# hi-paris/Prosody-Control-French-TTS

Measured on AMD Instinct MI355X. Metric: audio-seconds/sec prosody+align throughput, 16 kHz French, higher is better.
Workload: dtype fp16-resid16 (MFMA legs) + f64 (F0 / LUFS)

## Files before the change

include/pce.h:

```cpp
#ifndef PCE_H
#define PCE_H

#include <stddef.h>
#include <stdint.h>

#ifdef __cplusplus
extern "C" {
#endif

#pragma GCC visibility push(default)

#define PCE_API_VERSION 1
#define PCE_API_MINOR 6

typedef struct pce_ctx pce_ctx;

enum pce_status {
    PCE_OK = 0,
    PCE_E_INVALID = -1,
    PCE_E_DEVICE = -2,
    PCE_E_NOMEM = -3,
    PCE_E_STATE = -4,
    PCE_E_LIMIT = -5
};

enum pce_slice_status {
    PCE_SLICE_OK = 0,
    PCE_SLICE_TOO_SHORT = 1,
    PCE_SLICE_EMPTY = 2
};

typedef struct pce_slice {
    int32_t clip;
    int32_t flags;
    int64_t begin;
    int64_t end;
    double  x1;
} pce_slice;


pce_ctx *pce_create(int device, void *stream, char *err, size_t errlen);
void pce_destroy(pce_ctx *ctx);
const char *pce_last_error(const pce_ctx *ctx);
int pce_sync(pce_ctx *ctx);
int pce_api_version(void);
int pce_api_minor(void);
int pce_device_info(pce_ctx *ctx, char *name, size_t namelen, int32_t *compute_units, int64_t *hbm_bytes);

int pce_upload_pcm_s16(pce_ctx *ctx, const int16_t *pcm, const int64_t *offsets, int32_t n_clips, int32_t sample_rate);
int pce_bind_pcm_s16_device(pce_ctx *ctx, const void *d_pcm, const int64_t *offsets, int32_t n_clips, int32_t sample_rate);
int pce_num_clips(const pce_ctx *ctx);

int pce_resample_run(pce_ctx *ctx, int32_t up, int32_t down, const double *taps, int32_t n_taps, int64_t n_pre_remove);
int pce_download_pcm_s16(pce_ctx *ctx, int16_t *pcm, int64_t *offsets, int32_t *sample_rate);

int pce_frame_energy_run(pce_ctx *ctx, int32_t window, int32_t hop, int32_t requantize);
int pce_frame_energy_shape(pce_ctx *ctx, int32_t clip, int64_t *n_frames);
int pce_frame_energy_fetch(pce_ctx *ctx, int32_t clip, int64_t *sum_sq , int32_t *count );

typedef struct pce_energy {
    int64_t n;
    int64_t sum_sq;
    int64_t sum_sq_wrap16;
    int64_t n_loud;
    int32_t peak_abs;
    int32_t reserved;
} pce_energy;
int pce_energy_run(pce_ctx *ctx, const pce_slice *slices, int32_t n_slices, int32_t loud_threshold);
int pce_energy_fetch(pce_ctx *ctx, pce_energy *out );

int pce_lufs_set_meter_rate(pce_ctx *ctx, int32_t rate);
int pce_lufs_run(pce_ctx *ctx, const pce_slice *slices, int32_t n_slices);
int pce_lufs_fetch(pce_ctx *ctx, double *lufs , int32_t *status );

typedef struct pce_pitch_params {
    double  time_step;
    double  pitch_floor;
    double  periods_per_window;
    int32_t max_candidates;
    int32_t reserved;
    double  silence_threshold;
    double  voicing_threshold;
    double  octave_cost;
    double  octave_jump_cost;
    double  voiced_unvoiced_cost;
    double  pitch_ceiling;
} pce_pitch_params;

typedef struct pce_pitch_summary {
    int64_t n_frames;
    int64_t n_voiced;
    double  median_f0;
    double  mean_log_f0;
    double  t1;
    int32_t status;
    int32_t reserved;
} pce_pitch_summary;

int pce_pitch_plan(pce_ctx *ctx, const pce_pitch_params *p, const pce_slice *slices, int32_t n_slices,
                   int64_t *frame_offsets, int32_t *status);
int pce_pitch_run(pce_ctx *ctx, const pce_pitch_params *p, const pce_slice *slices, int32_t n_slices);
enum { PCE_REFINE_SEEDED = 0, PCE_REFINE_PRAAT = 1 };
int pce_pitch_set_refine(pce_ctx *ctx, int32_t mode);
int pce_pitch_fetch(pce_ctx *ctx, double *f0, double *strength, pce_pitch_summary *summary );

int pce_stft_db_run(pce_ctx *ctx, int32_t n_fft, int32_t hop);
int pce_stft_db_shape(pce_ctx *ctx, int32_t clip, int32_t *n_bins, int32_t *n_frames);
int pce_stft_db_fetch(pce_ctx *ctx, int32_t clip, float *out);
int pce_stft_db_device(pce_ctx *ctx, const void **d_ptr, int64_t *bytes);

typedef struct pce_pyin_plan {
    int32_t frame_length, hop_length, min_period, max_period, n_pitch_bins, trans_width, n_thresholds, reserved;
    double sr, fmin, bins_per_octave, no_trough_prob, log_tiny, log_p_init, tiny;
} pce_pyin_plan;
int pce_pyin_run(pce_ctx *ctx, const pce_pyin_plan *plan, const double *tables, int64_t n_tables);
int pce_pyin_shape(pce_ctx *ctx, int32_t clip, int64_t *n_frames);
int pce_pyin_fetch(pce_ctx *ctx, int32_t clip, int32_t *states, double *voiced_prob, int32_t *status);

typedef struct pce_whisper_dims {
    int32_t n_mels;
    int32_t n_ctx;
    int32_t n_state;
    int32_t n_head;
    int32_t n_layer;
} pce_whisper_dims;
int pce_logmel_run(pce_ctx *ctx, int32_t n_mels);
int pce_logmel_run_at(pce_ctx *ctx, int32_t n_mels, const int64_t *start_frames );
int pce_logmel_fetch(pce_ctx *ctx, int32_t clip, float *out );
int pce_whisper_load(pce_ctx *ctx, const pce_whisper_dims *dims, const float *weights, int64_t n_floats);
int pce_whisper_encode_run(pce_ctx *ctx);
int pce_selftest_gemm(pce_ctx *ctx, const uint16_t *A, const uint16_t *B, const float *bias, int32_t M, int32_t N, int32_t K, int32_t epilogue,
                      int32_t rows_per_clip, int32_t vt_sp, uint16_t *out);
int pce_selftest_attention(pce_ctx *ctx, const uint16_t *q, const uint16_t *k, const uint16_t *v, int32_t clips, int32_t heads, int32_t q_len,
                           int32_t k_len, int32_t causal, int32_t mode, uint16_t *out, int32_t *fell_back);
int pce_selftest_xattn(pce_ctx *ctx, const float *resid, const float *ln_w, const float *ln_b, const uint16_t *wq, const float *bq, const uint16_t *wk,
                       const uint16_t *wv, const float *bv, const uint16_t *E, const int32_t *k_len, int32_t n, int32_t k_cap, int32_t d, int32_t heads,
                       int32_t workgroups_per_clip, uint16_t *out);
int pce_selftest_gemm_tiled(pce_ctx *ctx, int32_t kernel, int32_t epilogue, const uint16_t *A, int64_t a_len, int64_t lda, int64_t a_batch, int32_t batch,
                            const uint16_t *B, const float *bias, int32_t M, int32_t N, int32_t K, void *C, int64_t c_len, int64_t ldc, int64_t c_batch,
                            const float *pos, int32_t pos_T, int32_t v_col0, int32_t rows_per_clip, int32_t vt_sp, uint16_t *vt, int64_t vt_len,
                            int32_t *kernel_used);
int pce_selftest_layernorm(pce_ctx *ctx, int32_t form, int32_t rows, int32_t d, const void *x, const uint16_t *delta, const uint16_t *delta2, const float *w,
                           const float *b, float eps, int32_t flags, void *out, void *resid_out, uint16_t *out_copy);
int pce_whisper_encode_fetch(pce_ctx *ctx, int32_t clip, float *out );

typedef struct pce_whisper_text_dims {
    int32_t n_vocab , n_text_ctx , n_state, n_head , n_layer;
} pce_whisper_text_dims;
int pce_whisper_decoder_load(pce_ctx *ctx, const pce_whisper_text_dims *dims, const float *weights, int64_t n_floats);
int pce_whisper_align_run(pce_ctx *ctx, const int32_t *tokens, const int32_t *token_offsets, const int32_t *num_frames,
                          int32_t sot_len, const uint8_t *head_mask, int32_t medfilt_width, float qk_scale);
int pce_whisper_align_shape(pce_ctx *ctx, int32_t clip, int32_t *n_rows, int32_t *n_cols);
int pce_whisper_align_fetch(pce_ctx *ctx, int32_t clip, int32_t *text_idx, int32_t *time_idx, int32_t *path_len, double *cost);
int pce_whisper_align_paths_enqueue(pce_ctx *ctx, int32_t slot, int32_t *n_clips, int32_t *path_stride);
int pce_whisper_align_paths_wait(pce_ctx *ctx, int32_t slot, int32_t *path_len, int32_t *text_idx, int32_t *time_idx);

typedef struct pce_whisper_decode_rules { int32_t eot, timestamp_begin, max_initial_timestamp_index , reserved; } pce_whisper_decode_rules;
int pce_whisper_decode_step(pce_ctx *ctx, const int32_t *tokens, const int32_t *token_offsets , int32_t sample_begin,
                            const pce_whisper_decode_rules *rules, const uint8_t *vocab_mask, int32_t *next_tokens ,
                            float *next_logprobs );
typedef struct pce_whisper_decode_opts {
    const int32_t *sample_begin;
    int32_t sample_begin_all;
    float temperature;
    uint32_t seed_lo, seed_hi;
    int32_t probe_token;
    int32_t flags;
} pce_whisper_decode_opts;
int pce_whisper_decode_step_ex(pce_ctx *ctx, const int32_t *tokens, const int32_t *token_offsets ,
                               const pce_whisper_decode_rules *rules, const uint8_t *vocab_mask, const pce_whisper_decode_opts *opts,
                               int32_t *next_tokens , float *next_logprobs ,
                               float *probe_prob );

int pce_whisper_sample_keys(pce_ctx *ctx, const int32_t *keys , int32_t n);

enum { PCE_OPERANDS_BF16 = 0, PCE_OPERANDS_FP16 = 1, PCE_OPERANDS_F16_RESID16 = 2 };
int pce_whisper_set_operands(pce_ctx *ctx, int32_t operand_type);
int pce_whisper_get_operands(pce_ctx *ctx);

int pce_whisper_decode_loop(pce_ctx *ctx, const int32_t *tokens, const int32_t *token_offsets ,
                            const pce_whisper_decode_rules *rules, const uint8_t *vocab_mask, const pce_whisper_decode_opts *opts,
                            int32_t max_new, int32_t check_every, int32_t *out_tokens, float *out_logprobs ,
                            int32_t *out_steps, float *probe_prob );

int pce_dtw(pce_ctx *ctx, const double *x, int32_t n_rows, int32_t n_cols, int32_t batch, int32_t *path_i, int32_t *path_j,
            int32_t *path_len);

#define PCE_DTW_SERIES_ROWS 1024
#define PCE_DTW_SERIES_COLS 2048
enum pce_dtw_status { PCE_DTW_OK = 0, PCE_DTW_EMPTY = 1, PCE_DTW_NO_PATH = 2 };
int pce_dtw_series(pce_ctx *ctx, const double *a, const int64_t *a_off, const double *b, const int64_t *b_off, const int32_t *win_lo,
                   const int32_t *win_hi, int32_t batch, int32_t *path_i, int32_t *path_j, int32_t *path_len, double *dist, int32_t *status);

int pce_nw_align(pce_ctx *ctx, const int32_t *a_ids, const int64_t *a_off, const int32_t *b_ids, const int64_t *b_off, int32_t batch,
                 int32_t match, int32_t mismatch, int32_t gap, int32_t *out_i, int32_t *out_j, int32_t *out_len);

int pce_levenshtein(pce_ctx *ctx, const uint32_t *a_chars, const int64_t *a_off, const uint32_t *b_chars, const int64_t *b_off,
                    int32_t batch, int32_t *out_dist);

typedef struct pce_bert_dims { int32_t n_vocab, n_pos, n_type, n_state, n_head, n_layer, n_labels; } pce_bert_dims;
int pce_bert_load(pce_ctx *ctx, const pce_bert_dims *dims, const float *weights, int64_t n_floats);
int pce_bert_run(pce_ctx *ctx, const int32_t *input_ids, const int32_t *offsets , int32_t n_seq);
int pce_bert_fetch(pce_ctx *ctx, int32_t seq, float *logits, int32_t *labels);

int pce_stats_enqueue(pce_ctx *ctx, int32_t slot);
int pce_stats_wait(pce_ctx *ctx, int32_t slot, pce_energy *energy, double *lufs, int32_t *lufs_status, pce_pitch_summary *pitch);

enum pce_kernel_id {
    PCE_K_ENERGY = 0,
    PCE_K_LUFS_PASS1, PCE_K_LUFS_SCAN, PCE_K_LUFS_PASS2, PCE_K_LUFS_GATE,
    PCE_K_PITCH_REFINE, PCE_K_PITCH_FRAMES, PCE_K_PITCH_PATH, PCE_K_PITCH_MEDIAN, PCE_K_PITCH_DELTA,
    PCE_K_STFT_MAX, PCE_K_STFT_DB, PCE_K_LOGMEL, PCE_K_WHISPER_ENC, PCE_K_RESAMPLE, PCE_K_DTW, PCE_K_WHISPER_ALIGN, PCE_K_NW, PCE_K_STFT_NORM,
    PCE_K_FRAME_ENERGY, PCE_K_BERT, PCE_K_PYIN_FRAMES, PCE_K_PYIN_VITERBI, PCE_K_WHISPER_DECODE,
    PCE_K_GEMM128, PCE_K_GEMM_WIDE, PCE_K_ATTENTION, PCE_K_LAYERNORM, PCE_K_GEMM_FLAT,
    PCE_K_ADD_LAYERNORM, PCE_K_STFT_RAW, PCE_K_LOGMEL_NORM, PCE_K_ATTENTION_LEAN,
// ... 17 lines not shown
```

prosody-control-french-tts_amd/csrc/pce_gemm256.inc:

```

constexpr int F_T = 256, F_K = 64, F_THREADS = 512;
constexpr int F_N_MAX = 6144;
constexpr bool F_PINGPONG = true;
constexpr int F_HALF = 128 * F_K;
constexpr int F_RING_BYTES = 8 * F_HALF * 2;
enum { FEPI_BF16 = 0, FEPI_GELU = 1, FEPI_VT = 2, FEPI_SPLIT = 3 };

__device__ __forceinline__ int f_swz(int row, int chunk) { return chunk ^ ((row >> 1) & 7); }
__device__ __forceinline__ int f_perm32(int p) { return ((p >> 2) & 3) * 8 + (p >> 4) * 4 + (p & 3); }

struct FCursor { int kofs, m0, n0, vt; };
struct FSched {
    int tiles_n, sm, sn, per_xcd, xcd, slot, wper, my_tiles;
    __device__ void init(int M, int N, int sm_, int sn_)
    {
        tiles_n = N / F_T; sm = sm_; sn = sn_;
        const int tiles_m = (M + F_T - 1) / F_T, tiles_m_pad = ((tiles_m + sm - 1) / sm) * sm;
        const int total = tiles_m_pad * tiles_n;
        per_xcd = (total + 7) >> 3; xcd = blockIdx.x & 7; slot = blockIdx.x >> 3; wper = gridDim.x >> 3;
        my_tiles = per_xcd > slot ? (per_xcd - slot + wper - 1) / wper : 0;
    }
    __device__ void tile(int it, int &m0, int &n0) const
    {
        const int lin = xcd * per_xcd + slot + it * wper;
        const int per = sm * sn, sup = lin / per, r = lin - sup * per;
        const int n_sn = tiles_n / sn;
        m0 = ((sup / n_sn) * sm + r / sn) * F_T; n0 = ((sup % n_sn) * sn + r % sn) * F_T;
    }
};

struct FFrags { opx8 RA[2][4], RB0[2][2], RB1[2][2]; };
struct FArgs {
    const op_t *A, *B; const float *bias; op_t *C;
    int M, N, K, ldc;
    int S, vt_sp;
    int sm, sn, stagger;
    op_t *C2; int vt_n0;
};

template <int N> __device__ __forceinline__ void f_wait_vm() { __builtin_amdgcn_s_waitcnt(((N >> 4) << 14) | 0x0F70 | (N & 15)); }
template <int N> __device__ __forceinline__ void f_wait_lgkm() { __builtin_amdgcn_s_waitcnt(0xC07F | (N << 8)); }

template <int KK, int HALF>
__device__ __forceinline__ void f_read_A(FFrags &F, const op_t *dsm, const int (&ra)[2], int par)
{
    const op_t *s = dsm + ((HALF ? 1 : 0) * 2 + par) * F_HALF;
#pragma unroll
    for (int i = 0; i < 4; i++) F.RA[KK][i] = *reinterpret_cast<const opx8 *>(s + ra[KK] + i * 16 * F_K);
}
template <int KK, int HALF>
__device__ __forceinline__ void f_read_B(FFrags &F, const op_t *dsm, const int (&rb)[2], int par)
{
    const op_t *s = dsm + ((HALF ? 1 : 0) * 2 + par) * F_HALF;
#pragma unroll
    for (int j = 0; j < 2; j++) {
        const opx8 v = *reinterpret_cast<const opx8 *>(s + rb[KK] + j * 16 * F_K);
        if (HALF) F.RB1[KK][j] = v; else F.RB0[KK][j] = v;
    }
}
template <bool VT, int HA, int HB, int KK, bool ZERO>
__device__ __forceinline__ void f_mma8(f32x4 (&acc)[2][2][4][2], const FFrags &F)
{
#pragma unroll
    for (int i = 0; i < 4; i++)
#pragma unroll
        for (int j = 0; j < 2; j++) {
            const opx8 b = HB ? F.RB1[KK][j] : F.RB0[KK][j];
            const f32x4 c = ZERO ? f32x4{0.f, 0.f, 0.f, 0.f} : acc[HA][HB][i][j];
            acc[HA][HB][i][j] = VT ? mfma16(F.RA[KK][i], b, c)
                                   : mfma16(b, F.RA[KK][i], c);
        }
}

template <int EPI>
__global__ __launch_bounds__(F_THREADS) __attribute__((amdgpu_waves_per_eu(2, 2))) void k_gemm_flat(FArgs P)
{
    constexpr bool SPLIT = EPI == FEPI_SPLIT;
    extern __shared__ __attribute__((aligned(1024))) op_t dsm[];
    float *sbias = reinterpret_cast<float *>(dsm + 8 * F_HALF);
    const int tid = threadIdx.x, lane = tid & 63, wv = __builtin_amdgcn_readfirstlane(tid >> 6);
    const int wr = wv >> 2, wc = wv & 3;
    const int fr = lane & 15, fq = lane >> 4;
    const int M = P.M, N = P.N, K = P.K;
    FSched S; S.init(M, N, P.sm, P.sn);
    const int nk = K / F_K;
    if (S.my_tiles == 0) return;
    for (int i = tid; i < N; i += F_THREADS) sbias[i] = P.bias ? P.bias[i] : 0.f;
    if (P.stagger > 0) {
        const unsigned long long t0 = __builtin_amdgcn_s_memtime(), d = (unsigned long long)P.stagger * (unsigned)(S.slot * 8 + S.xcd) / 256u;
        while (__builtin_amdgcn_s_memtime() - t0 < d) __builtin_amdgcn_s_sleep(8);
    }
    int voff_plain, voff_perm;
    {
        const int row = wv * 8 + (lane >> 3), c8 = f_swz(row, lane & 7) * 8;
        const int prow = (row & ~31) + f_perm32(row & 31);
        voff_plain = (row * K + c8) * 2; voff_perm = (prow * K + c8) * 2;
    }
    int ra[2], rb[2];
    {
        const int r_a = wr * 64 + fr, r_b = wc * 32 + fr;
        ra[0] = r_a * F_K + f_swz(r_a, fq) * 8; ra[1] = r_a * F_K + f_swz(r_a, 4 + fq) * 8;
        rb[0] = r_b * F_K + f_swz(r_b, fq) * 8 + 4 * F_HALF; rb[1] = r_b * F_K + f_swz(r_b, 4 + fq) * 8 + 4 * F_HALF;
    }
    const __amdgpu_buffer_rsrc_t rsA = __builtin_amdgcn_make_buffer_rsrc(const_cast<op_t *>(P.A), 0, (int)((unsigned)M * (unsigned)K * 2u), 0x00020000);
    const __amdgpu_buffer_rsrc_t rsB = __builtin_amdgcn_make_buffer_rsrc(const_cast<op_t *>(P.B), 0, (int)((unsigned)N * (unsigned)K * 2u), 0x00020000);
    const int ld2_64 = 64 * K * 2;
    FCursor pc1, pc2;
    int it1, kt1, it2, kt2;
    const int last_tile = S.my_tiles - 1;
    auto set_tile = [&](FCursor &c, int it) {
        S.tile(it < last_tile ? it : last_tile, c.m0, c.n0);
        c.vt = SPLIT ? (c.n0 >= P.vt_n0) : (EPI == FEPI_VT);
    };
    auto advance = [&](FCursor &c, int &it, int &kt) {
        if (++kt == nk) { kt = 0; ++it; set_tile(c, it); }
        c.kofs = kt * F_K;
    };
    auto issue = [&](const FCursor &c, int kind, int par) {
        op_t *slot = dsm + ((kind == 0 ? 0 : kind == 3 ? 1 : kind == 1 ? 2 : 3) * 2 + par) * F_HALF;
        const bool is_a = kind == 0 || kind == 3;
        const bool act = SPLIT ? (is_a != (c.vt != 0)) : is_a;
        const unsigned soff = (unsigned)((act ? c.m0 : c.n0) + ((kind == 3 || kind == 2) ? 128 : 0)) * (unsigned)K * 2u + (unsigned)c.kofs * 2u;
        const int voff = ((EPI == FEPI_VT) == is_a) ? voff_perm : voff_plain;
#pragma unroll
        for (int i = 0; i < 2; i++)
            __builtin_amdgcn_raw_ptr_buffer_load_lds(act ? rsA : rsB, (__attribute__((address_space(3))) void *)(slot + (wv + 8 * i) * 8 * F_K), 16,
                                                     voff, (int)(soff + (unsigned)(i * ld2_64)), 0, 0);
    };
    f32x4 acc[2][2][4][2];
#pragma unroll
    for (int a = 0; a < 2; a++)
#pragma unroll
        for (int b = 0; b < 2; b++)
#pragma unroll
            for (int i = 0; i < 4; i++)
#pragma unroll
                for (int j = 0; j < 2; j++) acc[a][b][i][j] = f32x4{0.f, 0.f, 0.f, 0.f};
    FFrags F;

#ifndef F_STORE_AUX
#define F_STORE_AUX 0
#endif
#define F_STORE_GUARD { asm volatile("s_nop 7\n\ts_nop 7" ::: "memory"); __builtin_amdgcn_sched_barrier(0); }
    typedef unsigned int u32x4 __attribute__((ext_vector_type(4)));
    constexpr bool HAS_RM = EPI != FEPI_VT, HAS_VT = EPI == FEPI_VT || SPLIT;
    const int Nv = SPLIT ? N - P.vt_n0 : N;
    op_t *const vt_ptr = SPLIT ? P.C2 : P.C;
    const __amdgpu_buffer_rsrc_t rsC = __builtin_amdgcn_make_buffer_rsrc(P.C, 0, HAS_RM ? (int)((unsigned)M * (unsigned)P.ldc * 2u) : 0, 0x00020000);
    const __amdgpu_buffer_rsrc_t rsV = __builtin_amdgcn_make_buffer_rsrc(vt_ptr, 0, HAS_VT ? (int)((unsigned)(M / P.S) * (unsigned)Nv * (unsigned)P.vt_sp * 2u) : 0, 0x00020000);
    const int voffC = (fr * P.ldc + fq * 8) * 2, voffV = (fr * P.vt_sp + fq * 8) * 2;
    auto store_rm = [&](int m0, int n0) {
#pragma unroll
        for (int hB = 0; hB < 2; hB++) {
            const float *bp = sbias + n0 + hB * 128 + wc * 32 + fq * 8;
            const float4 b0 = *reinterpret_cast<const float4 *>(bp), b1 = *reinterpret_cast<const float4 *>(bp + 4);
            const float bv[8] = {b0.x, b0.y, b0.z, b0.w, b1.x, b1.y, b1.z, b1.w};
#pragma unroll
            for (int hA = 0; hA < 2; hA++)
#pragma unroll
                for (int i = 0; i < 4; i++) {
                    opx8 o;
                    float t[8];
#pragma unroll
                    for (int e = 0; e < 8; e++) t[e] = acc[hA][hB][i][e >> 2][e & 3] + bv[e];
                    if (EPI == FEPI_GELU) gelu_exact8(t);
#pragma unroll
                    for (int e = 0; e < 8; e++) o[e] = (op_t)t[e];
                    const unsigned soff = ((unsigned)(m0 + hA * 128 + wr * 64 + i * 16) * (unsigned)P.ldc + (unsigned)(n0 + hB * 128 + wc * 32)) * 2u;
                    __builtin_amdgcn_raw_buffer_store_b128(__builtin_bit_cast(u32x4, o), rsC, voffC, (int)soff, F_STORE_AUX);
                    __builtin_amdgcn_sched_barrier(0);
                    F_STORE_GUARD
                }
        }
    };
    auto store_vt = [&](int m0, int n0, int nb0) {
        typedef __attribute__((ext_vector_type(4))) op_t opx4;
        typedef unsigned int u32x2 __attribute__((ext_vector_type(2)));
        const int clip0 = m0 / P.S, t_tile = m0 - clip0 * P.S;
        const int wrap = (Nv * P.vt_sp - P.S) * 2;
#pragma unroll
        for (int hB = 0; hB < 2; hB++)
#pragma unroll
            for (int j = 0; j < 2; j++) {
                const int n_s = n0 + hB * 128 + wc * 32 + j * 16;
                const float bv = sbias[nb0 + hB * 128 + wc * 32 + j * 16 + fr];
                const unsigned col = ((unsigned)clip0 * (unsigned)Nv + (unsigned)n_s) * (unsigned)P.vt_sp;
#pragma unroll
                for (int hA = 0; hA < 2; hA++)
#pragma unroll
                    for (int g = 0; g < 2; g++) {
                        const int t_g = t_tile + hA * 128 + wr * 64 + g * 32, rel = P.S - t_g;
                        if (!(rel > 0 && rel < 32 && (rel & 7) == 4)) {
                            opx8 o;
#pragma unroll
                            for (int r = 0; r < 8; r++) o[r] = (op_t)(acc[hA][hB][2 * g + (r >> 2)][j][r & 3] + bv);
                            const int voff = voffV + ((t_g + fq * 8 >= P.S) ? wrap : 0);
                            __builtin_amdgcn_raw_buffer_store_b128(__builtin_bit_cast(u32x4, o), rsV, voff, (int)((col + (unsigned)t_g) * 2u), F_STORE_AUX);
                            F_STORE_GUARD
                        } else {
#pragma unroll
                            for (int h = 0; h < 2; h++) {
                                const int t_s = t_g + h * 4;
                                opx4 o;
#pragma unroll
                                for (int r = 0; r < 4; r++) o[r] = (op_t)(acc[hA][hB][2 * g + h][j][r] + bv);
                                const int voff = voffV + ((t_s + fq * 8 >= P.S) ? wrap : 0);
                                __builtin_amdgcn_raw_buffer_store_b64(__builtin_bit_cast(u32x2, o), rsV, voff, (int)((col + (unsigned)t_s) * 2u), F_STORE_AUX);
                                F_STORE_GUARD
                            }
                        }
                    }
                __builtin_amdgcn_sched_barrier(0);
            }
    };
    auto store_vtT = [&](int m0, int n0) {
        typedef __attribute__((ext_vector_type(4))) op_t opx4;
        typedef unsigned int u32x2 __attribute__((ext_vector_type(2)));
        const int clip0 = m0 / P.S, t_tile = m0 - clip0 * P.S;
        const int wrap = (Nv * P.vt_sp - P.S) * 2;
#pragma unroll
        for (int hB = 0; hB < 2; hB++) {
            const int t_g = t_tile + hB * 128 + wc * 32, rel = P.S - t_g;
            const bool cut = rel > 0 && rel < 32 && (rel & 7) == 4;
#pragma unroll
            for (int hA = 0; hA < 2; hA++)
#pragma unroll
                for (int i = 0; i < 4; i++) {
                    const int n_r = hA * 128 + wr * 64 + i * 16;
                    const float bv = sbias[n0 + n_r + fr];
                    const unsigned base = (((unsigned)clip0 * (unsigned)Nv + (unsigned)(n0 - P.vt_n0 + n_r)) * (unsigned)P.vt_sp + (unsigned)t_g) * 2u;
                    if (!cut) {
                        opx8 o;
#pragma unroll
                        for (int e = 0; e < 8; e++) o[e] = (op_t)(acc[hA][hB][i][e >> 2][e & 3] + bv);
                        const int voff = voffV + ((t_g + fq * 8 >= P.S) ? wrap : 0);
                        __builtin_amdgcn_raw_buffer_store_b128(__builtin_bit_cast(u32x4, o), rsV, voff, (int)base, F_STORE_AUX);
                        F_STORE_GUARD
                    } else {
#pragma unroll
                        for (int h = 0; h < 2; h++) {
                            opx4 o;
#pragma unroll
                            for (int r = 0; r < 4; r++) o[r] = (op_t)(acc[hA][hB][i][h][r] + bv);
                            const int voff = voffV + h * 8 + ((t_g + fq * 8 + h * 4 >= P.S) ? wrap : 0);
                            __builtin_amdgcn_raw_buffer_store_b64(__builtin_bit_cast(u32x2, o), rsV, voff, (int)base, F_STORE_AUX);
                            F_STORE_GUARD
                        }
                    }
                    __builtin_amdgcn_sched_barrier(0);
                }
// ... 1 lines not shown
    };
    constexpr int EPI_OPS = 16;

    {
        FCursor c0; c0.kofs = 0; set_tile(c0, 0);
        it1 = 0; kt1 = 0; pc1 = c0; advance(pc1, it1, kt1);
        it2 = it1; kt2 = kt1; pc2 = pc1; advance(pc2, it2, kt2);
        __syncthreads();
        issue(c0, 0, 0); issue(c0, 1, 0); issue(c0, 2, 0); issue(c0, 3, 0);
        issue(pc1, 0, 1); issue(pc1, 1, 1); issue(pc1, 2, 1);
        f_wait_vm<6>();
        __builtin_amdgcn_s_barrier();
        if constexpr (!F_PINGPONG) {
            f_read_A<0, 0>(F, dsm, ra, 0); f_read_B<0, 0>(F, dsm, rb, 0); f_read_B<0, 1>(F, dsm, rb, 0); f_read_B<1, 1>(F, dsm, rb, 0);
            f_wait_lgkm<0>();
        }
    }
    int c_m0, c_n0;
    S.tile(0, c_m0, c_n0);
    int par = 0;
#define F_GROUP(HA, HB, KK) __builtin_amdgcn_s_setprio(1); f_mma8<VT, HA, HB, KK, false>(acc, F); \
                             __builtin_amdgcn_s_setprio(0); __builtin_amdgcn_sched_barrier(0);
#define F_ISSUE(C, KIND, PAR) __builtin_amdgcn_sched_barrier(0); issue(C, KIND, PAR); __builtin_amdgcn_sched_barrier(0);
    constexpr bool VT = EPI == FEPI_VT;
    auto kstep = [&](bool first_stores) {
        __builtin_amdgcn_s_barrier();
        F_ISSUE(pc1, 3, par ^ 1)
        f_read_A<1, 0>(F, dsm, ra, par); f_read_B<1, 0>(F, dsm, rb, par);
        f_wait_lgkm<6>(); F_GROUP(0, 0, 0)
        F_GROUP(0, 1, 0)
        f_read_A<0, 1>(F, dsm, ra, par);
        f_wait_lgkm<4>(); F_GROUP(0, 0, 1)
        F_GROUP(0, 1, 1)
        if (first_stores) f_wait_vm<2 + EPI_OPS>(); else f_wait_vm<2>();
        f_wait_lgkm<0>();
        __builtin_amdgcn_s_barrier();
        F_ISSUE(pc2, 0, par)
        f_read_A<1, 1>(F, dsm, ra, par);
        f_wait_lgkm<4>(); F_GROUP(1, 1, 0)
        F_ISSUE(pc2, 1, par)
        f_read_B<0, 1>(F, dsm, rb, par ^ 1);
        f_wait_lgkm<2>(); F_GROUP(1, 0, 0)
        F_ISSUE(pc2, 2, par)
        f_read_A<0, 0>(F, dsm, ra, par ^ 1); f_read_B<0, 0>(F, dsm, rb, par ^ 1);
        f_wait_lgkm<6>(); F_GROUP(1, 1, 1)
        f_read_B<1, 1>(F, dsm, rb, par ^ 1);
        f_wait_lgkm<2>(); F_GROUP(1, 0, 1)
    };
    auto kstep_pp = [&](int after_stores) {
        f_read_A<0, 0>(F, dsm, ra, par); f_read_A<1, 0>(F, dsm, ra, par); f_read_B<0, 0>(F, dsm, rb, par); f_read_B<1, 0>(F, dsm, rb, par);
        F_ISSUE(pc1, 3, par ^ 1)
        f_wait_lgkm<0>();
        __builtin_amdgcn_s_barrier();
        F_GROUP(0, 0, 0) F_GROUP(0, 0, 1)
        __builtin_amdgcn_s_barrier();
        f_read_B<0, 1>(F, dsm, rb, par); f_read_B<1, 1>(F, dsm, rb, par);
        F_ISSUE(pc2, 0, par)
        if (after_stores == 2) f_wait_vm<10>();
        f_wait_lgkm<0>();
        __builtin_amdgcn_s_barrier();
        F_GROUP(0, 1, 0) F_GROUP(0, 1, 1)
        __builtin_amdgcn_s_barrier();
        f_read_A<0, 1>(F, dsm, ra, par); f_read_A<1, 1>(F, dsm, ra, par);
        F_ISSUE(pc2, 1, par)
        f_wait_lgkm<0>();
        __builtin_amdgcn_s_barrier();
        F_GROUP(1, 1, 0) F_GROUP(1, 1, 1)
        __builtin_amdgcn_s_barrier();
        F_ISSUE(pc2, 2, par)
        if (after_stores == 1) f_wait_vm<8 + EPI_OPS>(); else f_wait_vm<6>();
        __builtin_amdgcn_s_barrier();
        F_GROUP(1, 0, 0) F_GROUP(1, 0, 1)
        __builtin_amdgcn_s_barrier();
    };
    if (F_PINGPONG && wr == 1) __builtin_amdgcn_s_barrier();
    for (int it = 0; it < S.my_tiles; it++) {
        const bool cur_vt = SPLIT ? (c_n0 >= P.vt_n0) : (EPI == FEPI_VT);
        for (int kt = 0; kt < nk; kt++) {
            const bool first = kt == 0, last = kt == nk - 1;
            if constexpr (F_PINGPONG) kstep_pp(it > 0 && nk >= 2 ? (kt == 0 ? 1 : kt == 1 ? 2 : 0) : 0);
            else kstep(first && it > 0);
            pc1 = pc2; it1 = it2; kt1 = kt2; advance(pc2, it2, kt2);
            if (last) {
                if (F_PINGPONG && wr == 0) __builtin_amdgcn_s_barrier();
                if constexpr (SPLIT) { if (cur_vt) store_vtT(c_m0, c_n0); else store_rm(c_m0, c_n0); }
                else if constexpr (EPI == FEPI_VT) store_vt(c_m0, c_n0, c_n0);
                else store_rm(c_m0, c_n0);
                if constexpr (!F_PINGPONG) f_wait_vm<6 + EPI_OPS>();
#pragma unroll
                for (int a = 0; a < 2; a++)
#pragma unroll
                    for (int b = 0; b < 2; b++)
#pragma unroll
                        for (int i = 0; i < 4; i++)
#pragma unroll
                            for (int j = 0; j < 2; j++) acc[a][b][i][j] = f32x4{0.f, 0.f, 0.f, 0.f};
                if (F_PINGPONG && wr == 1) __builtin_amdgcn_s_barrier();
            } else if constexpr (!F_PINGPONG) f_wait_vm<6>();
            f_wait_lgkm<0>();
            par ^= 1;
        }
        if (it + 1 < S.my_tiles) S.tile(it + 1, c_m0, c_n0);
    }
    if (F_PINGPONG && wr == 0) __builtin_amdgcn_s_barrier();
    f_wait_vm<0>();
#undef F_GROUP
#undef F_ISSUE
#undef F_STORE_GUARD
}

template <class OUT, class RIN, class ROUT, int NV = 5>
__global__ __launch_bounds__(256) void k_add_layernorm(const RIN *resid_in, ROUT *resid_out, const op_t *__restrict__ delta, const op_t *__restrict__ delta2,
                                                      int write_resid, const float *__restrict__ w,
                                                      const float *__restrict__ b, int64_t rows, int d, OUT *__restrict__ out, float eps,
                                                      op_t *__restrict__ out_bf16 = nullptr )
{
    constexpr bool IN16 = !std::is_same<RIN, float>::value, OUT16 = !std::is_same<ROUT, float>::value;
    const int64_t row = (int64_t)blockIdx.x * 4 + (threadIdx.x >> 6);
    const int lane = threadIdx.x & 63;
    if (row >= rows) return;
    typedef __attribute__((ext_vector_type(4))) op_t opx4;
    const opx4 *dr = reinterpret_cast<const opx4 *>(delta + row * d);
    const opx4 *dr2 = reinterpret_cast<const opx4 *>(delta2 ? delta2 + row * d : nullptr);
    auto r16 = [](float x) -> float { return OUT16 ? (float)(op_t)x : x; };
    const int nv = d >> 2;
    float4 v[NV];
    float s = 0.f;
#pragma unroll
    for (int i = 0; i < NV; i++) {
        const int idx = lane + 64 * i;
        if (idx < nv) {
            f32x4 x;
            if constexpr (IN16) {
                const opx4 xh = __builtin_nontemporal_load(reinterpret_cast<const opx4 *>(resid_in + row * d) + idx);
                x = f32x4{(float)xh[0], (float)xh[1], (float)xh[2], (float)xh[3]};
            } else {
                x = __builtin_nontemporal_load(reinterpret_cast<const f32x4 *>(resid_in + row * d) + idx);
                if constexpr (OUT16) x = f32x4{r16(x[0]), r16(x[1]), r16(x[2]), r16(x[3])};
            }
            const opx4 dl = __builtin_nontemporal_load(dr + idx);
            v[i] = make_float4(r16(x[0] + (float)dl[0]), r16(x[1] + (float)dl[1]), r16(x[2] + (float)dl[2]), r16(x[3] + (float)dl[3]));
            if (dr2) {
                const opx4 d2 = __builtin_nontemporal_load(dr2 + idx);
                v[i] = make_float4(r16(v[i].x + (float)d2[0]), r16(v[i].y + (float)d2[1]), r16(v[i].z + (float)d2[2]), r16(v[i].w + (float)d2[3]));
            }
            if (write_resid) {
                if constexpr (OUT16) {
                    opx4 o; o[0] = (op_t)v[i].x; o[1] = (op_t)v[i].y; o[2] = (op_t)v[i].z; o[3] = (op_t)v[i].w;
                    __builtin_nontemporal_store(o, reinterpret_cast<opx4 *>(resid_out + row * d) + idx);
                } else __builtin_nontemporal_store(f32x4{v[i].x, v[i].y, v[i].z, v[i].w}, reinterpret_cast<f32x4 *>(resid_out + row * d) + idx);
            }
        } else v[i] = make_float4(0.f, 0.f, 0.f, 0.f);
        s += (v[i].x + v[i].y) + (v[i].z + v[i].w);
    }
    s = wave_allsum_f32(s);
    const float mean = s / (float)d;
    float q = 0.f;
#pragma unroll
    for (int i = 0; i < NV; i++) {
        if (lane + 64 * i < nv) {
            const float a0 = v[i].x - mean, a1 = v[i].y - mean, a2 = v[i].z - mean, a3 = v[i].w - mean;
            q += (a0 * a0 + a1 * a1) + (a2 * a2 + a3 * a3);
        }
    }
    q = wave_allsum_f32(q);
    const float inv = rsqrtf(q / (float)d + eps);
// ... 13 lines not shown
```

prosody-control-french-tts_amd/csrc/pce_whisper_dispatch.hip:

```cpp
#include "pce_internal.h"

#define PCE_BOTH(ret, name, params)  extern "C" { ret name##_bf16 params; ret name##_f16 params; }
#define PCE_FWD(name, ...) ((c && c->whisper_ops >= 1) ? name##_f16(__VA_ARGS__) : name##_bf16(__VA_ARGS__))

PCE_BOTH(int, pce_logmel_run, (pce_ctx *, int32_t))
PCE_BOTH(int, pce_logmel_run_at, (pce_ctx *, int32_t, const int64_t *))
PCE_BOTH(int, pce_logmel_fetch, (pce_ctx *, int32_t, float *))
PCE_BOTH(int, pce_whisper_load, (pce_ctx *, const pce_whisper_dims *, const float *, int64_t))
PCE_BOTH(int, pce_whisper_encode_run, (pce_ctx *))
PCE_BOTH(int, pce_whisper_encode_fetch, (pce_ctx *, int32_t, float *))
PCE_BOTH(int, pce_selftest_attention, (pce_ctx *, const uint16_t *, const uint16_t *, const uint16_t *, int32_t, int32_t, int32_t, int32_t, int32_t, int32_t, uint16_t *, int32_t *))
PCE_BOTH(int, pce_selftest_gemm, (pce_ctx *, const uint16_t *, const uint16_t *, const float *, int32_t, int32_t, int32_t, int32_t, int32_t, int32_t, uint16_t *))
PCE_BOTH(int, pce_selftest_xattn, (pce_ctx *, const float *, const float *, const float *, const uint16_t *, const float *, const uint16_t *, const uint16_t *, const float *, const uint16_t *, const int32_t *, int32_t, int32_t, int32_t, int32_t, int32_t, uint16_t *))
PCE_BOTH(int, pce_selftest_gemm_tiled, (pce_ctx *, int32_t, int32_t, const uint16_t *, int64_t, int64_t, int64_t, int32_t, const uint16_t *, const float *, int32_t, int32_t,
                                         int32_t, void *, int64_t, int64_t, int64_t, const float *, int32_t, int32_t, int32_t, int32_t, uint16_t *, int64_t, int32_t *))
PCE_BOTH(int, pce_selftest_layernorm, (pce_ctx *, int32_t, int32_t, int32_t, const void *, const uint16_t *, const uint16_t *, const float *, const float *, float, int32_t,
                                        void *, void *, uint16_t *))
PCE_BOTH(int, pce_whisper_decoder_load, (pce_ctx *, const pce_whisper_text_dims *, const float *, int64_t))
PCE_BOTH(int, pce_whisper_align_run, (pce_ctx *, const int32_t *, const int32_t *, const int32_t *, int32_t, const uint8_t *, int32_t, float))
PCE_BOTH(int, pce_whisper_align_fetch, (pce_ctx *, int32_t, int32_t *, int32_t *, int32_t *, double *))
PCE_BOTH(int, pce_whisper_align_shape, (pce_ctx *, int32_t, int32_t *, int32_t *))
PCE_BOTH(int, pce_whisper_align_paths_enqueue, (pce_ctx *, int32_t, int32_t *, int32_t *))
PCE_BOTH(int, pce_whisper_align_paths_wait, (pce_ctx *, int32_t, int32_t *, int32_t *, int32_t *))
PCE_BOTH(int, pce_whisper_sample_keys, (pce_ctx *, const int32_t *, int32_t))
PCE_BOTH(int, pce_whisper_decode_step, (pce_ctx *, const int32_t *, const int32_t *, int32_t, const pce_whisper_decode_rules *, const uint8_t *, int32_t *, float *))
PCE_BOTH(int, pce_whisper_decode_step_ex, (pce_ctx *, const int32_t *, const int32_t *, const pce_whisper_decode_rules *, const uint8_t *, const pce_whisper_decode_opts *, int32_t *, float *, float *))
PCE_BOTH(int, pce_whisper_decode_loop, (pce_ctx *, const int32_t *, const int32_t *, const pce_whisper_decode_rules *, const uint8_t *, const pce_whisper_decode_opts *, int32_t, int32_t, int32_t *, float *, int32_t *, float *))
PCE_BOTH(int, pce_bert_load, (pce_ctx *, const pce_bert_dims *, const float *, int64_t))
PCE_BOTH(int, pce_bert_run, (pce_ctx *, const int32_t *, const int32_t *, int32_t))
PCE_BOTH(int, pce_bert_fetch, (pce_ctx *, int32_t, float *, int32_t *))
void pce_whisper_free_bf16(pce_ctx *c);
void pce_whisper_free_f16(pce_ctx *c);

void pce_whisper_free(pce_ctx *c) { pce_whisper_free_bf16(c); pce_whisper_free_f16(c); }

extern "C" {

int pce_whisper_set_operands(pce_ctx *c, int32_t operand_type)
{
    if (!c) return PCE_E_INVALID;
    if (operand_type != PCE_OPERANDS_BF16 && operand_type != PCE_OPERANDS_FP16 && operand_type != PCE_OPERANDS_F16_RESID16)
        return pce_fail(c, PCE_E_INVALID, "operand type %d (0 = bf16, 1 = fp16, 2 = fp16 with the fp16 residual stream)", operand_type);
    c->whisper_ops = operand_type;
    c->resid16 = operand_type == PCE_OPERANDS_F16_RESID16;
    return PCE_OK;
}
int pce_whisper_get_operands(pce_ctx *c) { return c ? c->whisper_ops : PCE_E_INVALID; }

int pce_logmel_run(pce_ctx *c, int32_t n_mels) { return PCE_FWD(pce_logmel_run, c, n_mels); }
int pce_logmel_run_at(pce_ctx *c, int32_t n_mels, const int64_t *start_frames) { return PCE_FWD(pce_logmel_run_at, c, n_mels, start_frames); }
int pce_logmel_fetch(pce_ctx *c, int32_t clip, float *out) { return PCE_FWD(pce_logmel_fetch, c, clip, out); }
int pce_whisper_load(pce_ctx *c, const pce_whisper_dims *dims, const float *weights, int64_t n_floats) { return PCE_FWD(pce_whisper_load, c, dims, weights, n_floats); }
int pce_whisper_encode_run(pce_ctx *c) { return PCE_FWD(pce_whisper_encode_run, c); }
int pce_whisper_encode_fetch(pce_ctx *c, int32_t clip, float *out) { return PCE_FWD(pce_whisper_encode_fetch, c, clip, out); }
int pce_selftest_attention(pce_ctx *c, const uint16_t *q, const uint16_t *k, const uint16_t *v, int32_t clips, int32_t heads, int32_t q_len, int32_t k_len,
                           int32_t causal, int32_t mode, uint16_t *out, int32_t *fell_back)
{
    return PCE_FWD(pce_selftest_attention, c, q, k, v, clips, heads, q_len, k_len, causal, mode, out, fell_back);
}
int pce_selftest_gemm(pce_ctx *c, const uint16_t *A, const uint16_t *B, const float *bias, int32_t M, int32_t N, int32_t K, int32_t epilogue, int32_t rows_per_clip,
                      int32_t vt_sp, uint16_t *out)
{
    return PCE_FWD(pce_selftest_gemm, c, A, B, bias, M, N, K, epilogue, rows_per_clip, vt_sp, out);
}
int pce_selftest_xattn(pce_ctx *c, const float *resid, const float *ln_w, const float *ln_b, const uint16_t *wq, const float *bq, const uint16_t *wk, const uint16_t *wv,
                       const float *bv, const uint16_t *E, const int32_t *k_len, int32_t n, int32_t k_cap, int32_t d, int32_t heads, int32_t workgroups_per_clip, uint16_t *out)
{
    return PCE_FWD(pce_selftest_xattn, c, resid, ln_w, ln_b, wq, bq, wk, wv, bv, E, k_len, n, k_cap, d, heads, workgroups_per_clip, out);
}
int pce_selftest_gemm_tiled(pce_ctx *c, int32_t kernel, int32_t epilogue, const uint16_t *A, int64_t a_len, int64_t lda, int64_t a_batch, int32_t batch,
                            const uint16_t *B, const float *bias, int32_t M, int32_t N, int32_t K, void *C, int64_t c_len, int64_t ldc, int64_t c_batch,
                            const float *pos, int32_t pos_T, int32_t v_col0, int32_t rows_per_clip, int32_t vt_sp, uint16_t *vt, int64_t vt_len, int32_t *kernel_used)
{
    return PCE_FWD(pce_selftest_gemm_tiled, c, kernel, epilogue, A, a_len, lda, a_batch, batch, B, bias, M, N, K, C, c_len, ldc, c_batch, pos, pos_T, v_col0,
                   rows_per_clip, vt_sp, vt, vt_len, kernel_used);
}
int pce_selftest_layernorm(pce_ctx *c, int32_t form, int32_t rows, int32_t d, const void *x, const uint16_t *delta, const uint16_t *delta2, const float *w,
                           const float *b, float eps, int32_t flags, void *out, void *resid_out, uint16_t *out_copy)
{
    return PCE_FWD(pce_selftest_layernorm, c, form, rows, d, x, delta, delta2, w, b, eps, flags, out, resid_out, out_copy);
}
int pce_whisper_decoder_load(pce_ctx *c, const pce_whisper_text_dims *dims, const float *weights, int64_t n_floats)
{
    return PCE_FWD(pce_whisper_decoder_load, c, dims, weights, n_floats);
}
int pce_whisper_align_run(pce_ctx *c, const int32_t *tokens, const int32_t *token_offsets, const int32_t *num_frames, int32_t sot_len, const uint8_t *head_mask,
                          int32_t medfilt_width, float qk_scale)
{
    return PCE_FWD(pce_whisper_align_run, c, tokens, token_offsets, num_frames, sot_len, head_mask, medfilt_width, qk_scale);
}
int pce_whisper_align_fetch(pce_ctx *c, int32_t clip, int32_t *text_idx, int32_t *time_idx, int32_t *path_len, double *cost)
{
    return PCE_FWD(pce_whisper_align_fetch, c, clip, text_idx, time_idx, path_len, cost);
}
int pce_whisper_align_shape(pce_ctx *c, int32_t clip, int32_t *n_rows, int32_t *n_cols) { return PCE_FWD(pce_whisper_align_shape, c, clip, n_rows, n_cols); }
int pce_whisper_align_paths_enqueue(pce_ctx *c, int32_t slot, int32_t *n_clips, int32_t *path_stride) { return PCE_FWD(pce_whisper_align_paths_enqueue, c, slot, n_clips, path_stride); }
int pce_whisper_align_paths_wait(pce_ctx *c, int32_t slot, int32_t *path_len, int32_t *text_idx, int32_t *time_idx)
{
    return PCE_FWD(pce_whisper_align_paths_wait, c, slot, path_len, text_idx, time_idx);
}
int pce_whisper_sample_keys(pce_ctx *c, const int32_t *keys, int32_t n) { return PCE_FWD(pce_whisper_sample_keys, c, keys, n); }
int pce_whisper_decode_step(pce_ctx *c, const int32_t *tokens, const int32_t *token_offsets, int32_t sample_begin, const pce_whisper_decode_rules *rules,
                            const uint8_t *vocab_mask, int32_t *next_tokens, float *next_logprobs)
{
    return PCE_FWD(pce_whisper_decode_step, c, tokens, token_offsets, sample_begin, rules, vocab_mask, next_tokens, next_logprobs);
}
int pce_whisper_decode_step_ex(pce_ctx *c, const int32_t *tokens, const int32_t *token_offsets, const pce_whisper_decode_rules *rules, const uint8_t *vocab_mask,
                               const pce_whisper_decode_opts *opts, int32_t *next_tokens, float *next_logprobs, float *probe_prob)
{
    return PCE_FWD(pce_whisper_decode_step_ex, c, tokens, token_offsets, rules, vocab_mask, opts, next_tokens, next_logprobs, probe_prob);
}
int pce_whisper_decode_loop(pce_ctx *c, const int32_t *tokens, const int32_t *token_offsets, const pce_whisper_decode_rules *rules, const uint8_t *vocab_mask,
                            const pce_whisper_decode_opts *opts, int32_t max_new, int32_t check_every, int32_t *out_tokens, float *out_logprobs, int32_t *out_steps,
                            float *probe_prob)
{
    return PCE_FWD(pce_whisper_decode_loop, c, tokens, token_offsets, rules, vocab_mask, opts, max_new, check_every, out_tokens, out_logprobs, out_steps, probe_prob);
}
int pce_bert_load(pce_ctx *c, const pce_bert_dims *dims, const float *weights, int64_t n_floats) { return PCE_FWD(pce_bert_load, c, dims, weights, n_floats); }
int pce_bert_run(pce_ctx *c, const int32_t *input_ids, const int32_t *offsets, int32_t n_seq) { return PCE_FWD(pce_bert_run, c, input_ids, offsets, n_seq); }
int pce_bert_fetch(pce_ctx *c, int32_t seq, float *logits, int32_t *labels) { return PCE_FWD(pce_bert_fetch, c, seq, logits, labels); }

}
```

prosody-control-french-tts_amd/csrc/pce_whisper_impl.inc:

```
#include "pce_internal.h"
#include <cmath>
#include <cstdlib>
#include <type_traits>

#define pce_logmel_run PCE_WFN(pce_logmel_run)
#define pce_logmel_run_at PCE_WFN(pce_logmel_run_at)
#define pce_logmel_fetch PCE_WFN(pce_logmel_fetch)
#define pce_whisper_load PCE_WFN(pce_whisper_load)
#define pce_whisper_encode_run PCE_WFN(pce_whisper_encode_run)
#define pce_whisper_encode_fetch PCE_WFN(pce_whisper_encode_fetch)
#define pce_selftest_attention PCE_WFN(pce_selftest_attention)
#define pce_selftest_gemm PCE_WFN(pce_selftest_gemm)
#define pce_whisper_decoder_load PCE_WFN(pce_whisper_decoder_load)
#define pce_whisper_align_run PCE_WFN(pce_whisper_align_run)
#define pce_whisper_align_fetch PCE_WFN(pce_whisper_align_fetch)
#define pce_whisper_align_shape PCE_WFN(pce_whisper_align_shape)
#define pce_whisper_align_paths_enqueue PCE_WFN(pce_whisper_align_paths_enqueue)
#define pce_whisper_align_paths_wait PCE_WFN(pce_whisper_align_paths_wait)
#define pce_whisper_sample_keys PCE_WFN(pce_whisper_sample_keys)
#define pce_whisper_decode_step PCE_WFN(pce_whisper_decode_step)
#define pce_whisper_decode_step_ex PCE_WFN(pce_whisper_decode_step_ex)
#define pce_whisper_decode_loop PCE_WFN(pce_whisper_decode_loop)
#define pce_bert_load PCE_WFN(pce_bert_load)
#define pce_bert_run PCE_WFN(pce_bert_run)
#define pce_bert_fetch PCE_WFN(pce_bert_fetch)
#define pce_selftest_xattn PCE_WFN(pce_selftest_xattn)
#define pce_selftest_gemm_tiled PCE_WFN(pce_selftest_gemm_tiled)
#define pce_selftest_layernorm PCE_WFN(pce_selftest_layernorm)
#define pce_whisper_free PCE_WFN(pce_whisper_free)
extern "C" int pce_whisper_decode_step_ex(pce_ctx *c, const int32_t *tokens, const int32_t *token_offsets, const pce_whisper_decode_rules *rules,
                                          const uint8_t *vocab_mask, const pce_whisper_decode_opts *opts, int32_t *next_tokens,
                                          float *next_logprobs, float *probe_prob);
void pce_whisper_free(pce_ctx *c);

namespace {

typedef PCE_OP_T op_t;
typedef __attribute__((ext_vector_type(8))) op_t opx8;
typedef __attribute__((ext_vector_type(4))) float f32x4;

template <class T> struct MfmaOf;
template <> struct MfmaOf<__bf16> {
    typedef __attribute__((ext_vector_type(8))) __bf16 v8;
    static __device__ __forceinline__ f32x4 m16(v8 a, v8 b, f32x4 c) { return __builtin_amdgcn_mfma_f32_16x16x32_bf16(a, b, c, 0, 0, 0); }
};
template <> struct MfmaOf<_Float16> {
    typedef __attribute__((ext_vector_type(8))) _Float16 v8;
    static __device__ __forceinline__ f32x4 m16(v8 a, v8 b, f32x4 c) { return __builtin_amdgcn_mfma_f32_16x16x32_f16(a, b, c, 0, 0, 0); }
};
__device__ __forceinline__ f32x4 mfma16(opx8 a, opx8 b, f32x4 c) { return MfmaOf<op_t>::m16(a, b, c); }

constexpr int W_NFFT = 400, W_HOP = 160, W_BINS = 201, W_FRAMES = 3000, W_SAMPLES = 480000;
constexpr int W_CTX = 1500;
constexpr double W_PI = 3.14159265358979323846;

struct MelTables {
    const float2 *w16;
    const float2 *w400;
    const float2 *w25;
    const float *window;
    const int *mel_lo;
    const int *mel_n;
    const int *mel_off;
    const float *mel_w;
    int mel_total;
};

__device__ __forceinline__ unsigned int f32_order_key(float f)
{
    const unsigned int b = __float_as_uint(f);
    return (b & 0x80000000u) ? ~b : (b | 0x80000000u);
}
__device__ __forceinline__ float f32_from_key(unsigned int k)
{
    return __uint_as_float((k & 0x80000000u) ? (k & 0x7FFFFFFFu) : ~k);
}

constexpr int LM_MELW = 1024;
template <int LM_G>
__global__ __launch_bounds__(256) PCE_NO_PK_F32 void k_logmel_frames(const int16_t *__restrict__ pcm, const int64_t *__restrict__ clip_off, int n_mels,
                                                      MelTables T, float *__restrict__ logspec ,
                                                      unsigned int *__restrict__ clip_max, const int64_t *__restrict__ frame0, int scan)
{
    __shared__ float xs[4][W_NFFT];
    __shared__ float2 ys[4][25 * 16];
    __shared__ float pw[4][W_BINS + 3];
    __shared__ float2 s_w16[16], s_w25[25], s_w400[25 * 16];
    __shared__ float s_melw[LM_MELW];
    const int tid = threadIdx.x, lane = tid & 63, wv = tid >> 6;
    for (int i = tid; i < T.mel_total; i += 256) s_melw[i] = T.mel_w[i];
    for (int i = tid; i < 16; i += 256) s_w16[i] = T.w16[i];
    for (int i = tid; i < 25; i += 256) s_w25[i] = T.w25[i];
    for (int i = tid; i < 400; i += 256) s_w400[i] = T.w400[i];
    __syncthreads();
    const int clip = blockIdx.y;
// ... 502 lines not shown
#pragma unroll
    for (int s = 0; s < W_STAGES - 1; s++)
        if (s < nk) {
            stage_rows32<G_BM>(A, lda, m0, M - 1, s * W_BK, smem + s * W_STAGE, wv, lane);
            stage_rows32<W_BN>(B, K, n0, N - 1, s * W_BK, smem + s * W_STAGE + G_BM * W_BK, wv, lane);
        }
    int cur = 0;
    for (int kt = 0; kt < nk; kt++) {
        const op_t *sA = smem + cur * W_STAGE, *sB = sA + G_BM * W_BK;
        if (W_STAGES > 2 && kt + 1 < nk) asm volatile("s_waitcnt vmcnt(3)" ::: "memory");
        else asm volatile("s_waitcnt vmcnt(0)" ::: "memory");
        __builtin_amdgcn_s_barrier();
        if (kt + W_STAGES - 1 < nk) {
            int nx = cur + W_STAGES - 1; if (nx >= W_STAGES) nx -= W_STAGES;
            op_t *nA = smem + nx * W_STAGE;
            stage_rows32<G_BM>(A, lda, m0, M - 1, (kt + W_STAGES - 1) * W_BK, nA, wv, lane);
            stage_rows32<W_BN>(B, K, n0, N - 1, (kt + W_STAGES - 1) * W_BK, nA + G_BM * W_BK, wv, lane);
        }
        opx8 a[4], b[4];
#pragma unroll
        for (int i = 0; i < 4; i++) {
            const int row = wr * 64 + i * 16 + fr;
            a[i] = *reinterpret_cast<const opx8 *>(&sA[row * W_BK + swz32(row, fq) * 8]);
        }
#pragma unroll
        for (int j = 0; j < 4; j++) {
            const int row = wc * 64 + j * 16 + fr;
            b[j] = *reinterpret_cast<const opx8 *>(&sB[row * W_BK + swz32(row, fq) * 8]);
        }
#pragma unroll
        for (int i = 0; i < 4; i++)
#pragma unroll
            for (int j = 0; j < 4; j++) acc[i][j] = mfma16(a[i], b[j], acc[i][j]);
        cur = cur + 1 == W_STAGES ? 0 : cur + 1;
    }
    float *tile = reinterpret_cast<float *>(smem);
#pragma unroll
    for (int p = 0; p < 2; p++) {
        __syncthreads();
        if ((wc >> 1) == p) {
#pragma unroll
            for (int i = 0; i < 4; i++)
#pragma unroll
                for (int j = 0; j < 4; j++)
#pragma unroll
                    for (int r = 0; r < 4; r++)
                        tile[(wr * 64 + i * 16 + fq * 4 + r) * G_TLD + (wc & 1) * 64 + j * 16 + fr] = acc[i][j][r];
        }
        __syncthreads();
        if (p == 0) gemm_store_tile<EPI>(tile, tid, m0, n0, M, N, bv0, bc0, Cv, ldc, (int64_t)blockIdx.z * c_batch, pos, pos_T, v_col0, vt_sp);
        else gemm_store_tile<EPI>(tile, tid, m0, n0 + 128, M, N, bv1, bc1, Cv, ldc, (int64_t)blockIdx.z * c_batch, pos, pos_T, v_col0, vt_sp);
    }
}

template <class OUT> __device__ __forceinline__ void ln_store4(OUT *p, float a, float b, float c, float d);
template <> __device__ __forceinline__ void ln_store4<float>(float *p, float a, float b, float c, float d)
{
    *reinterpret_cast<float4 *>(p) = make_float4(a, b, c, d);
}
template <> __device__ __forceinline__ void ln_store4<op_t>(op_t *p, float a, float b, float c, float d)
{
    typedef __attribute__((ext_vector_type(4))) op_t opx4;
    opx4 v; v[0] = (op_t)a; v[1] = (op_t)b; v[2] = (op_t)c; v[3] = (op_t)d;
    *reinterpret_cast<opx4 *>(p) = v;
}

template <int CTRL> __device__ __forceinline__ float dpp_f32(float v)
{
    return __builtin_bit_cast(float, __builtin_amdgcn_update_dpp(0, __builtin_bit_cast(int, v), CTRL, 0xF, 0xF, true));
}
__device__ __forceinline__ float wave_allsum_f32(float v)
{
    v += dpp_f32<0xB1>(v);
    v += dpp_f32<0x4E>(v);
    v += dpp_f32<0x141>(v);
    v += dpp_f32<0x140>(v);
    const int b = __builtin_bit_cast(int, v);
    const float r0 = __builtin_bit_cast(float, __builtin_amdgcn_readlane(b, 0)), r1 = __builtin_bit_cast(float, __builtin_amdgcn_readlane(b, 16));
    const float r2 = __builtin_bit_cast(float, __builtin_amdgcn_readlane(b, 32)), r3 = __builtin_bit_cast(float, __builtin_amdgcn_readlane(b, 48));
    return (r0 + r1) + (r2 + r3);
}

constexpr int LN_D_MAX = 2048;
template <class OUT, int NV = 5>
__global__ __launch_bounds__(256) void k_layernorm(const float *x, const float *__restrict__ w, const float *__restrict__ b,
                                                  int64_t rows, int d, OUT *__restrict__ out, float eps = 1e-5f, float *out2 = nullptr, int round_in16 = 0)
{
    const int64_t row = (int64_t)blockIdx.x * 4 + (threadIdx.x >> 6);
    const int lane = threadIdx.x & 63;
    if (row >= rows) return;
    const float4 *xr = reinterpret_cast<const float4 *>(x + row * d);
    const int nv = d >> 2;
    float4 v[NV];
    float s = 0.f;
#pragma unroll
    for (int i = 0; i < NV; i++) {
        const int idx = lane + 64 * i;
        v[i] = idx < nv ? xr[idx] : make_float4(0.f, 0.f, 0.f, 0.f);
        if (round_in16) v[i] = make_float4((float)(op_t)v[i].x, (float)(op_t)v[i].y, (float)(op_t)v[i].z, (float)(op_t)v[i].w);
        s += (v[i].x + v[i].y) + (v[i].z + v[i].w);
    }
    s = wave_allsum_f32(s);
    const float mean = s / (float)d;
    float q = 0.f;
#pragma unroll
    for (int i = 0; i < NV; i++) {
        if (lane + 64 * i < nv) {
            const float a0 = v[i].x - mean, a1 = v[i].y - mean, a2 = v[i].z - mean, a3 = v[i].w - mean;
            q += (a0 * a0 + a1 * a1) + (a2 * a2 + a3 * a3);
        }
    }
    q = wave_allsum_f32(q);
    const float inv = rsqrtf(q / (float)d + eps);
#pragma unroll
    for (int i = 0; i < NV; i++) {
        const int idx = lane + 64 * i;
        if (idx < nv) {
            const float4 ww = reinterpret_cast<const float4 *>(w)[idx], bb = reinterpret_cast<const float4 *>(b)[idx];
            const float y0 = (v[i].x - mean) * inv * ww.x + bb.x, y1 = (v[i].y - mean) * inv * ww.y + bb.y,
                        y2 = (v[i].z - mean) * inv * ww.z + bb.z, y3 = (v[i].w - mean) * inv * ww.w + bb.w;
            ln_store4<OUT>(out + row * d + 4 * idx, y0, y1, y2, y3);
            if (out2) ln_store4<float>(out2 + row * d + 4 * idx, y0, y1, y2, y3);
        }
    }
}

#include "pce_gemm256.inc"

constexpr int AT_QB = 128;

struct AttnArgs {
    const op_t *q; int64_t q_ld;
    const op_t *k; int64_t k_ld;
    const op_t *vt; int64_t vt_clip; int vt_sp;
    const int *q_row0, *q_len, *k_row0, *k_len;
    op_t *out; int64_t out_ld;
    int causal;
    int *fell_back;
};

template <bool EXACT, bool NT>
__device__ __forceinline__ bool attn_block16(const AttnArgs &A, op_t *smem, int bx, int head, int clip)
{
    constexpr int NS = 3, DPW = 4;
    const int tid = threadIdx.x, lane = tid & 63, wv = __builtin_amdgcn_readfirstlane(tid >> 6);
    const int n16 = lane & 15, g = lane >> 4;
    const int Sq = A.q_len[clip], Sk = A.k_len[clip];
    const int q0 = bx * AT_QB + wv * 32;
    const op_t *qbase = A.q + (int64_t)A.q_row0[clip] * A.q_ld + head * 64;
    const op_t *kbase = A.k + (int64_t)A.k_row0[clip] * A.k_ld + head * 64;
    const op_t *vtbase = A.vt + (int64_t)clip * A.vt_clip + (int64_t)head * 64 * A.vt_sp;
    const int kld = (int)A.k_ld, vsp = A.vt_sp;
    const __amdgpu_buffer_rsrc_t rsK = __builtin_amdgcn_make_buffer_rsrc(const_cast<op_t *>(kbase), 0, ((Sk - 1) * kld + 64) * 2, 0x00020000);
    const __amdgpu_buffer_rsrc_t rsV = __builtin_amdgcn_make_buffer_rsrc(const_cast<op_t *>(vtbase), 0, 64 * vsp * 2, 0x00020000);
    int voffK[2], voffV[2];
#pragma unroll
    for (int i = 0; i < 2; i++) {
        const int row = (wv + 4 * i) * 8 + (lane >> 3), c8 = swz_chunk(row, lane & 7) * 8;
        const int kb = row >> 4, rho = row & 15;
        const int key = 32 * (kb >> 1) + 8 * (rho >> 2) + 4 * (kb & 1) + (rho & 3);
        voffK[i] = (key * kld + c8) * 2; voffV[i] = (row * vsp + c8) * 2;
    }
    auto stage = [&](int t) {
        op_t *sK = smem + (t % NS) * (2 * 64 * 64), *sV = sK + 64 * 64;
        const int key0 = t * 64;
#pragma unroll
        for (int i = 0; i < 2; i++) {
            __builtin_amdgcn_raw_ptr_buffer_load_lds(rsK, (__attribute__((address_space(3))) void *)(sK + (wv + 4 * i) * 8 * 64), 16, voffK[i], key0 * kld * 2, 0, NT ? 3 : 0);
            __builtin_amdgcn_raw_ptr_buffer_load_lds(rsV, (__attribute__((address_space(3))) void *)(sV + (wv + 4 * i) * 8 * 64), 16, voffV[i], key0 * 2, 0, NT ? 3 : 0);
        }
    };
    const f32x4 z4 = {0.f, 0.f, 0.f, 0.f};
    opx8 qf[2][2];
    int my_q[2];
#pragma unroll
    for (int qb = 0; qb < 2; qb++) {
        my_q[qb] = q0 + 16 * qb + n16;
        int qr = my_q[qb]; if (qr >= Sq) qr = Sq - 1;
        const op_t *qp = qbase + (int64_t)qr * A.q_ld;
#pragma unroll
        for (int ks = 0; ks < 2; ks++) qf[qb][ks] = *reinterpret_cast<const opx8 *>(qp + 32 * ks + 8 * g);
    }
    opx8 ones;
#pragma unroll
    for (int j = 0; j < 8; j++) ones[j] = (op_t)(n16 == 0 ? 1.0f : 0.0f);
    f32x4 o[4][2], osum[2];
#pragma unroll
    for (int db = 0; db < 4; db++) { o[db][0] = z4; o[db][1] = z4; }
    osum[0] = z4; osum[1] = z4;
    float m_run[2] = {-1e30f, -1e30f}, l_run[2] = {0.f, 0.f};
    const float sl2 = 0.125f * 1.4426950408889634f;
    int k_need = Sk;
    if (A.causal) k_need = min(Sk, bx * AT_QB + AT_QB);
    const int nt = (k_need + 63) / 64;
    int kaddr[4][2], vaddr[4][2];
#pragma unroll
    for (int b4 = 0; b4 < 4; b4++)
#pragma unroll
        for (int ks = 0; ks < 2; ks++) {
            const int row = 16 * b4 + n16;
            kaddr[b4][ks] = row * 64 + swz_chunk(row, 4 * ks + g) * 8;
            vaddr[b4][ks] = 64 * 64 + row * 64 + swz_chunk(row, 4 * ks + g) * 8;
        }
    stage(0);
    if (nt > 1) stage(1);
// ... 925 lines not shown
    P.sn = 1;
    for (int cand : {4, 3, 2}) if (tiles_n % cand == 0) { P.sn = cand; break; }
    const int tiles_m = (M + F_T - 1) / F_T;
    int sm_want = 16;
    P.stagger = 20000;
    if (tiles_n == 3 && K <= 1024) { P.sn = 1; sm_want = 8; }
    else if (tiles_n == 6) P.sn = tiles_n;
    P.sm = tiles_m < sm_want ? tiles_m : sm_want;
    const int lds = F_RING_BYTES + N * (int)sizeof(float);
    const int grid = ((c->cu_count > 0 ? c->cu_count : 256) / 8) * 8;
    KernelTimer kt(c, prof_id, nullptr, 2.0 * M * (double)N * K);
    hipLaunchKernelGGL((k_gemm_flat<EPI>), dim3((unsigned)grid), dim3(F_THREADS), lds, c->stream, P);
    return true;
}

enum GemmKernel { GK_AUTO = 0, GK_SKINNY = 1, GK_WIDE = 2, GK_128 = 3, GK_128_DEEP = 4 };
struct GemmShape { int M, N, K; int64_t lda; int batch; int v_col0; };
template <int EPI> static bool gemm_fits(int kind, const GemmShape &s)
{
    switch (kind) {
    case GK_SKINNY:
        return (EPI == EPI_BF16 || EPI == EPI_GELU_BF16 || EPI == EPI_RESID_F32) && s.batch == 1 && s.M <= 1024 && s.N <= 4096 && s.N % S_BN == 0 &&
               s.K % S_KC == 0 && s.lda % 8 == 0;
    case GK_WIDE: return s.N % W_BN == 0 && s.K % W_BK == 0 && (EPI != EPI_QKV || s.v_col0 % W_BN == 0);
    case GK_128: case GK_128_DEEP: return s.N % G_BN == 0 && s.K % G_BK == 0 && (EPI != EPI_QKV || s.v_col0 % G_BN == 0);
    default: return false;
    }
}
template <int EPI> static int gemm_choose(const pce_ctx *c, const GemmShape &s)
{
    if (c->gemm_skinny && c->gemm_few_rows && gemm_fits<EPI>(GK_SKINNY, s)) return GK_SKINNY;
    if (gemm_fits<EPI>(GK_WIDE, s) && s.N >= 1536 && !(EPI == EPI_F32 && (int64_t)s.M * s.batch <= 1024))
        return GK_WIDE;
    if ((int64_t)s.M * s.batch <= 1024 && s.K >= 4 * G_BK) return GK_128_DEEP;
    return GK_128;
}
template <int EPI>
static void launch_gemm_kernel(pce_ctx *c, int kind, const op_t *A, int64_t lda, int64_t a_batch, const op_t *B, int M, int N, int K, const float *bias,
                               void *C, int64_t ldc, int64_t c_batch, int batch, const float *pos, int pos_T, int v_col0, int vt_sp)
{
    if constexpr (EPI == EPI_BF16 || EPI == EPI_GELU_BF16 || EPI == EPI_RESID_F32) {
        if (kind == GK_SKINNY) {
            KernelTimer kt(c, PCE_K_GEMM_SKINNY, nullptr, 2.0 * M * (double)N * K);
            hipLaunchKernelGGL((k_gemm_skinny<EPI>), dim3((unsigned)(N / S_BN), (unsigned)div_up(M, S_BM)), dim3(S_THREADS), S_LDS, c->stream,
                               A, lda, B, M, N, K, bias, C, ldc);
            return;
        }
    }
    if (kind == GK_WIDE) {
        const int wt = N / W_BN;
        int wsn = 1;
        for (int cand : {4, 3, 2}) if (wt % cand == 0) { wsn = cand; break; }
        const int wsm = 16;
        dim3 wgrid((unsigned)wt, (unsigned)(div_up(M, G_BM * wsm) * wsm), (unsigned)batch);
        KernelTimer kt(c, PCE_K_GEMM_WIDE, nullptr, 2.0 * M * (double)N * K * batch);
        hipLaunchKernelGGL((k_gemm_wide<EPI>), wgrid, dim3(G_THREADS), 0, c->stream, A, lda, a_batch, B, M, N, K, bias, C, ldc, c_batch, pos, pos_T,
                           v_col0, vt_sp, wsn, wsm);
        return;
    }
    const int tiles_n = N / G_BN;
    int sn = 1;
    for (int cand : {8, 6, 4, 3, 2}) if (tiles_n % cand == 0) { sn = cand; break; }
    const int sm = 16;
    dim3 grid((unsigned)tiles_n, (unsigned)(div_up(M, G_BM * sm) * sm), (unsigned)batch);
    KernelTimer kt(c, PCE_K_GEMM128, nullptr, 2.0 * M * (double)N * K * batch);
    if (kind == GK_128_DEEP)
        hipLaunchKernelGGL((k_gemm_bf16<EPI, 4>), grid, dim3(G_THREADS), 0, c->stream, A, lda, a_batch, B, M, N, K, bias, C, ldc, c_batch, pos, pos_T,
                           v_col0, vt_sp, sn, sm);
    else
        hipLaunchKernelGGL((k_gemm_bf16<EPI>), grid, dim3(G_THREADS), 0, c->stream, A, lda, a_batch, B, M, N, K, bias, C, ldc, c_batch, pos, pos_T,
                           v_col0, vt_sp, sn, sm);
}
template <int EPI>
void launch_gemm(pce_ctx *c, const op_t *A, int64_t lda, int64_t a_batch, const op_t *B, int M, int N, int K, const float *bias,
                 void *C, int64_t ldc, int64_t c_batch, int batch, const float *pos = nullptr, int pos_T = 1, int v_col0 = 0,
                 int vt_sp = AT_SP)
{
    const int kind = gemm_choose<EPI>(c, GemmShape{M, N, K, lda, batch, v_col0});
    launch_gemm_kernel<EPI>(c, kind, A, lda, a_batch, B, M, N, K, bias, C, ldc, c_batch, batch, pos, pos_T, v_col0, vt_sp);
}

template <class OUT>
static void launch_layernorm(pce_ctx *c, const float *x, const float *w, const float *b, int64_t rows, int d, OUT *out, float eps = 1e-5f,
                             float *out2 = nullptr, int round_in16 = 0)
{
    const dim3 grid((unsigned)div_up(rows, 4)), block(256);
    if (d <= 1280) hipLaunchKernelGGL((k_layernorm<OUT, 5>), grid, block, 0, c->stream, x, w, b, rows, d, out, eps, out2, round_in16);
    else hipLaunchKernelGGL((k_layernorm<OUT, 8>), grid, block, 0, c->stream, x, w, b, rows, d, out, eps, out2, round_in16);
}
template <class OUT, class RIN, class ROUT>
static void launch_add_layernorm(pce_ctx *c, const RIN *resid_in, ROUT *resid_out, const op_t *delta, const op_t *delta2, int write_resid, const float *w,
                                 const float *b, int64_t rows, int d, OUT *out, float eps, op_t *out_bf16)
{
    const dim3 grid((unsigned)div_up(rows, 4)), block(256);
    if (d <= 1280)
        hipLaunchKernelGGL((k_add_layernorm<OUT, RIN, ROUT, 5>), grid, block, 0, c->stream, resid_in, resid_out, delta, delta2, write_resid, w, b, rows, d, out, eps, out_bf16);
    else
        hipLaunchKernelGGL((k_add_layernorm<OUT, RIN, ROUT, 8>), grid, block, 0, c->stream, resid_in, resid_out, delta, delta2, write_resid, w, b, rows, d, out, eps, out_bf16);
}

static bool xa_has_form(int d, int heads)
{
    return heads * 64 == d && (d == 128 || d == 256 || d == 384 || d == 512 || d == 768 || d == 1024 || d == 1280);
}
static int xa_split(int n, int wpc) { return (wpc == 1 || wpc == 2 || wpc == 4) ? wpc : n >= 512 ? 1 : n >= 256 ? 2 : 4; }
template <int D> struct XaWidth {
    static constexpr int NSLOT = (D == 512 || D == 768 || D == 1024) ? 2 : 3, WV = xa_waves(D), RT = D > 1024 ? 2 : 1;
    static constexpr bool PAIRS = D <= 768;
    static constexpr size_t LDS = xa_lds(D, NSLOT);
};
struct XaLayer {
    const float *resid, *ln_w, *ln_b, *bq, *bv;
    const op_t *wq, *wkT, *wv;
    op_t *qp_hi, *qp_lo, *out; int64_t out_ld;
};
template <int D>
static void xattn_launch_d(pce_ctx *c, int n, XaArgs a, const XaLayer &y)
{
    using W = XaWidth<D>;
    a.qp_hi = y.qp_hi; a.qp_lo = y.qp_lo;
    const dim3 hgrid((unsigned)a.heads, (unsigned)div_up(n, 16)), grid((unsigned)(n * a.nsplit)), block(64 * (unsigned)W::WV);
    hipLaunchKernelGGL(k_xq_fused<D>, hgrid, dim3(256), 0, c->stream, y.resid, y.ln_w, y.ln_b, y.wq, y.bq, y.wkT, n, 0.125f * 1.4426950408889634f, a.skip,
                       y.qp_hi, y.qp_lo, a.rows);
    auto uv = [&](auto kern) {
        hipLaunchKernelGGL(kern, hgrid, dim3(256), 0, c->stream, a.u_part, a.ml_part, y.wv, y.bv, n, a.skip, y.out, y.out_ld, a.rows);
    };
    if constexpr (W::PAIRS) {
        if (a.nsplit <= XA_LEAVES / 2) {
            hipLaunchKernelGGL((k_xattn_absorbed<D, W::NSLOT, true, W::WV, W::RT>), grid, block, W::LDS, c->stream, a);
            uv(k_uv_absorb<D, true>);
            return;
        }
    }
    hipLaunchKernelGGL((k_xattn_absorbed<D, W::NSLOT, false, W::WV, W::RT>), grid, block, W::LDS, c->stream, a);
    uv(k_uv_absorb<D, false>);
}
static void xattn_launch(pce_ctx *c, int d, int n, const XaArgs &a, const XaLayer &y)
{
    switch (d) {
    case 128: xattn_launch_d<128>(c, n, a, y); break;
    case 256: xattn_launch_d<256>(c, n, a, y); break;
    case 384: xattn_launch_d<384>(c, n, a, y); break;
    case 512: xattn_launch_d<512>(c, n, a, y); break;
    case 768: xattn_launch_d<768>(c, n, a, y); break;
    case 1024: xattn_launch_d<1024>(c, n, a, y); break;
    default: xattn_launch_d<1280>(c, n, a, y); break;
    }
}

template <int D> static hipError_t xattn_optin()
{
    using W = XaWidth<D>;
    if constexpr (W::PAIRS) {
        const hipError_t e = hipFuncSetAttribute((const void *)k_xattn_absorbed<D, W::NSLOT, true, W::WV, W::RT>, hipFuncAttributeMaxDynamicSharedMemorySize, (int)W::LDS);
        if (e != hipSuccess) return e;
    }
    return hipFuncSetAttribute((const void *)k_xattn_absorbed<D, W::NSLOT, false, W::WV, W::RT>, hipFuncAttributeMaxDynamicSharedMemorySize, (int)W::LDS);
}
static int lds_optins(pce_ctx *c, WhisperState *w)
{
    if (w->lds_opted_in) return PCE_OK;
    const hipFuncAttribute A = hipFuncAttributeMaxDynamicSharedMemorySize;
    const int flat = F_RING_BYTES + F_N_MAX * (int)sizeof(float);
    PCE_HIP(c, hipFuncSetAttribute((const void *)k_gemm_flat<FEPI_BF16>, A, flat));
    PCE_HIP(c, hipFuncSetAttribute((const void *)k_gemm_flat<FEPI_GELU>, A, flat));
    PCE_HIP(c, hipFuncSetAttribute((const void *)k_gemm_flat<FEPI_VT>, A, flat));
    PCE_HIP(c, hipFuncSetAttribute((const void *)k_gemm_flat<FEPI_SPLIT>, A, flat));
    PCE_HIP(c, hipFuncSetAttribute((const void *)k_gemm_skinny<EPI_BF16>, A, S_LDS));
    PCE_HIP(c, hipFuncSetAttribute((const void *)k_gemm_skinny<EPI_GELU_BF16>, A, S_LDS));
    PCE_HIP(c, hipFuncSetAttribute((const void *)k_gemm_skinny<EPI_RESID_F32>, A, S_LDS));
    PCE_HIP(c, hipFuncSetAttribute((const void *)k_cross_attn1w, A, 16 * 1600 * 4));
    PCE_HIP(c, xattn_optin<128>()); PCE_HIP(c, xattn_optin<256>()); PCE_HIP(c, xattn_optin<384>()); PCE_HIP(c, xattn_optin<512>());
    PCE_HIP(c, xattn_optin<768>()); PCE_HIP(c, xattn_optin<1024>()); PCE_HIP(c, xattn_optin<1280>());
    w->lds_opted_in = true;
    return PCE_OK;
}

template <int EPI> static int selftest_gemm_kind(const pce_ctx *c, int kernel, const GemmShape &s)
{
    const int kind = kernel == GK_AUTO ? gemm_choose<EPI>(c, s) : kernel;
    return gemm_fits<EPI>(kind, s) ? kind : -1;
}

template <class OUT, class RIN, class ROUT>
static int selftest_add_layernorm(pce_ctx *c, int64_t rows, int d, const void *x, const uint16_t *delta, const uint16_t *delta2, const float *w, const float *b,
                                  float eps, int write_resid, void *out, void *resid_out, uint16_t *out_copy)
{
    constexpr bool IN_PLACE = std::is_same<RIN, ROUT>::value;
    const size_t n = (size_t)rows * d;
    DevBuf din, dres, ddl, ddl2, dw, db, dout, dcopy;
    PCE_HIP(c, din.reserve(sizeof(RIN) * n)); PCE_HIP(c, ddl.reserve(2 * n)); PCE_HIP(c, dw.reserve(sizeof(float) * d)); PCE_HIP(c, db.reserve(sizeof(float) * d));
    PCE_HIP(c, dout.reserve(sizeof(OUT) * n));
    if (!IN_PLACE) PCE_HIP(c, dres.reserve(sizeof(ROUT) * n));
    if (delta2) PCE_HIP(c, ddl2.reserve(2 * n));
    if (out_copy) PCE_HIP(c, dcopy.reserve(2 * n));
    PCE_HIP(c, hipMemcpyAsync(din.p, x, sizeof(RIN) * n, hipMemcpyHostToDevice, c->stream));
    PCE_HIP(c, hipMemcpyAsync(ddl.p, delta, 2 * n, hipMemcpyHostToDevice, c->stream));
    if (delta2) PCE_HIP(c, hipMemcpyAsync(ddl2.p, delta2, 2 * n, hipMemcpyHostToDevice, c->stream));
    PCE_HIP(c, hipMemcpyAsync(dw.p, w, sizeof(float) * d, hipMemcpyHostToDevice, c->stream));
    PCE_HIP(c, hipMemcpyAsync(db.p, b, sizeof(float) * d, hipMemcpyHostToDevice, c->stream));
    PCE_HIP(c, hipMemsetAsync(dout.p, 0, sizeof(OUT) * n, c->stream));
    if (!IN_PLACE) PCE_HIP(c, hipMemsetAsync(dres.p, 0, sizeof(ROUT) * n, c->stream));
    if (out_copy) PCE_HIP(c, hipMemsetAsync(dcopy.p, 0, 2 * n, c->stream));
    ROUT *rout = IN_PLACE ? din.as<ROUT>() : dres.as<ROUT>();
    launch_add_layernorm<OUT, RIN, ROUT>(c, din.as<RIN>(), rout, ddl.as<op_t>(), delta2 ? ddl2.as<op_t>() : nullptr, write_resid, dw.as<float>(), db.as<float>(),
                                         rows, d, dout.as<OUT>(), eps, out_copy ? dcopy.as<op_t>() : nullptr);
    PCE_HIP(c, hipGetLastError());
    PCE_HIP(c, hipMemcpyAsync(out, dout.p, sizeof(OUT) * n, hipMemcpyDeviceToHost, c->stream));
    if (resid_out) PCE_HIP(c, hipMemcpyAsync(resid_out, rout, sizeof(ROUT) * n, hipMemcpyDeviceToHost, c->stream));
    if (out_copy) PCE_HIP(c, hipMemcpyAsync(out_copy, dcopy.p, 2 * n, hipMemcpyDeviceToHost, c->stream));
    PCE_HIP(c, hipStreamSynchronize(c->stream));
    return PCE_OK;
}

}

void pce_whisper_free(pce_ctx *c)
{
    if (!c->whisper_slot[PCE_OP_INDEX]) return;
    WhisperState *w = static_cast<WhisperState *>(c->whisper_slot[PCE_OP_INDEX]);
    for (auto &ps : w->al_slot) {
        if (ps.host) (void)hipHostFree(ps.host);
        if (ps.ev) (void)hipEventDestroy(ps.ev);
    }
    delete w;
    c->whisper_slot[PCE_OP_INDEX] = nullptr;
}

extern "C" {

static int logmel_run_impl(pce_ctx *c, int32_t n_mels, const int64_t *start_frames);
int pce_logmel_run(pce_ctx *c, int32_t n_mels) { return logmel_run_impl(c, n_mels, nullptr); }
int pce_logmel_run_at(pce_ctx *c, int32_t n_mels, const int64_t *start_frames)
{
    if (!start_frames) return PCE_E_INVALID;
    return logmel_run_impl(c, n_mels, start_frames);
}
static int logmel_run_impl(pce_ctx *c, int32_t n_mels, const int64_t *start_frames)
{
    if (!c) return PCE_E_INVALID;
    if (!c->d_pcm) return pce_fail(c, PCE_E_STATE, "no batch uploaded");
    if (c->rate != 16000) return pce_fail(c, PCE_E_INVALID, "log-mel needs 16 kHz audio (got %d Hz): resample on the host first", c->rate);
    if (n_mels <= 0 || n_mels > 128) return pce_fail(c, PCE_E_INVALID, "n_mels %d out of range", n_mels);
    PCE_HIP(c, hipSetDevice(c->device));
    WhisperState *w = ws_of(c);
    int rc = mel_setup(c, w, n_mels);
    if (rc) return rc;
    const int32_t n = c->n_clips;
    const size_t tm_elems = (size_t)n * (W_FRAMES + 2) * (size_t)n_mels + 512;
    PCE_HIP(c, w->logspec.reserve(sizeof(float) * (size_t)n * (size_t)n_mels * W_FRAMES));
// ... 112 lines not shown
        ly.ln2_w = add_vec(p, (size_t)d); p += d; ly.ln2_b = add_vec(p, (size_t)d); p += d;
        ly.m1_w = mats.size(); mats.insert(mats.end(), p, p + (size_t)4 * d * d); p += (size_t)4 * d * d;
        ly.m1_b = add_vec(p, (size_t)4 * d); p += 4 * d;
        ly.m2_w = mats.size(); mats.insert(mats.end(), p, p + (size_t)4 * d * d); p += (size_t)4 * d * d;
        ly.m2_b = add_vec(p, (size_t)d); p += d;
    }
    w->lnp_w = add_vec(p, (size_t)d); p += d; w->lnp_b = add_vec(p, (size_t)d); p += d;
    std::vector<float> pos((size_t)W_CTX * d);
    {
        const int half = d / 2;
        const double inc = std::log(10000.0) / (half - 1);
        for (int t = 0; t < W_CTX; t++)
            for (int i = 0; i < half; i++) {
                const float inv = (float)std::exp(-inc * i);
                const float a = (float)t * inv;
                pos[(size_t)t * d + i] = std::sin(a); pos[(size_t)t * d + half + i] = std::cos(a);
            }
    }
    DevBuf tmp;
    PCE_HIP(c, tmp.reserve(sizeof(float) * mats.size()));
    PCE_HIP(c, w->w_bf16.reserve(sizeof(op_t) * mats.size() + 256));
    PCE_HIP(c, w->w_f32.reserve(sizeof(float) * vecs.size()));
    PCE_HIP(c, w->pos.reserve(sizeof(float) * pos.size()));
    PCE_HIP(c, hipMemcpyAsync(tmp.p, mats.data(), sizeof(float) * mats.size(), hipMemcpyHostToDevice, c->stream));
    PCE_HIP(c, hipMemcpyAsync(w->w_f32.p, vecs.data(), sizeof(float) * vecs.size(), hipMemcpyHostToDevice, c->stream));
    PCE_HIP(c, hipMemcpyAsync(w->pos.p, pos.data(), sizeof(float) * pos.size(), hipMemcpyHostToDevice, c->stream));
    hipLaunchKernelGGL(k_f32_to_bf16, dim3((unsigned)div_up((int64_t)mats.size(), 256)), dim3(256), 0, c->stream, tmp.as<float>(),
                       w->w_bf16.as<op_t>(), (int64_t)mats.size());
    PCE_HIP(c, hipStreamSynchronize(c->stream));
    w->loaded = true;
    return PCE_OK;
}

int pce_whisper_encode_run(pce_ctx *c)
{
    if (!c) return PCE_E_INVALID;
    WhisperState *w = ws_of(c);
    if (!w->loaded) return pce_fail(c, PCE_E_STATE, "pce_whisper_encode_run before pce_whisper_load");
    if (w->n_clips_mel < 0 || w->mel_nmels != w->dims.n_mels) return pce_fail(c, PCE_E_STATE, "run pce_logmel_run(n_mels of the model) first");
    PCE_HIP(c, hipSetDevice(c->device));
    const int d = w->dims.n_state, L = w->dims.n_layer, nm = w->dims.n_mels, H = w->dims.n_head;
    const int n = w->n_clips_mel;
    const int64_t M = (int64_t)n * W_CTX;
    if (M > INT32_MAX) return pce_fail(c, PCE_E_LIMIT, "too many clips for one encoder batch");
    const int K1p = (int)div_up(3 * nm, 64) * 64;
    const size_t c1_elems = (size_t)n * (W_FRAMES + 2) * (size_t)d + 4096;
    PCE_HIP(c, w->c1_out.reserve(sizeof(op_t) * c1_elems));
    PCE_HIP(c, w->resid.reserve(sizeof(float) * (size_t)M * d));
    PCE_HIP(c, w->ln_out.reserve(sizeof(op_t) * (size_t)M * d));
    PCE_HIP(c, w->qkv.reserve(sizeof(op_t) * (size_t)M * 2 * d));
    const size_t vt_elems = (size_t)n * (size_t)d * AT_SP + 64;
    {
        const size_t before = w->vt.cap;
        PCE_HIP(c, w->vt.reserve(sizeof(op_t) * vt_elems));
        if (w->vt.cap != before || w->vt_elems_zeroed < vt_elems) {
            PCE_HIP(c, hipMemsetAsync(w->vt.p, 0, sizeof(op_t) * vt_elems, c->stream));
            w->vt_elems_zeroed = vt_elems;
        }
    }
    PCE_HIP(c, w->attn.reserve(sizeof(op_t) * (size_t)M * d));
    PCE_HIP(c, w->hidden.reserve(sizeof(op_t) * (size_t)M * 4 * d));
    PCE_HIP(c, w->final_out.reserve(sizeof(float) * (size_t)M * d));
    const op_t *Wb = w->w_bf16.as<op_t>();
    const float *Wf = w->w_f32.as<float>();
    if (w->enc_tab_clips != n) {
        std::vector<int> tab((size_t)2 * n);
        for (int i = 0; i < n; i++) { tab[(size_t)i] = i * W_CTX; tab[(size_t)n + i] = W_CTX; }
        PCE_HIP(c, w->enc_tab.reserve(sizeof(int) * tab.size()));
        PCE_HIP(c, hipMemcpyAsync(w->enc_tab.p, tab.data(), sizeof(int) * tab.size(), hipMemcpyHostToDevice, c->stream));
        PCE_HIP(c, hipStreamSynchronize(c->stream));
        w->enc_tab_clips = n;
    }
    KernelTimer t(c, PCE_K_WHISPER_ENC);
    if (w->c1_out.cap != w->c1_zero_cap || w->c1_zero_d != d) {
        PCE_HIP(c, hipMemsetAsync(w->c1_out.p, 0, w->c1_out.cap, c->stream));
        w->c1_zero_cap = w->c1_out.cap; w->c1_zero_d = d;
    }
    launch_gemm<EPI_GELU_BF16>(c, w->mel_tm.as<op_t>(), nm, (int64_t)(W_FRAMES + 2) * nm, Wb + w->c1_w, W_FRAMES, d, K1p, Wf + w->c1_b,
                               w->c1_out.as<op_t>() + d, d, (int64_t)(W_FRAMES + 2) * d, n);
    launch_gemm<EPI_GELU_POS_F32>(c, w->c1_out.as<op_t>(), 2 * (int64_t)d, (int64_t)(W_FRAMES + 2) * d, Wb + w->c2_w, W_CTX, d, 3 * d,
                                  Wf + w->c2_b, w->resid.as<float>(), d, (int64_t)W_CTX * d, n, w->pos.as<float>(), W_CTX);
    const bool flat = c->gemm_flat && d % F_T == 0 && gemm_flat_offsets_fit(M, 4 * d, 4 * d, 4 * d, 0, 0) &&
                      gemm_flat_offsets_fit(M, d, d, 0, W_CTX, AT_SP);
    if (flat) {
        PCE_HIP(c, w->delta.reserve(sizeof(op_t) * (size_t)M * d)); PCE_HIP(c, w->delta2.reserve(sizeof(op_t) * (size_t)M * d));
        PCE_HIP(c, w->d_enc_bf16.reserve(sizeof(op_t) * (size_t)M * d + 4096));
    }
    const bool resid16 = flat && c->resid16 && PCE_OP_INDEX == 1;
    if (resid16) PCE_HIP(c, w->resid16.reserve(sizeof(op_t) * (size_t)M * d));
    auto add_ln = [&](size_t w_off, size_t b_off, bool mid, bool last, bool first_layer) {
        KernelTimer kt(c, PCE_K_ADD_LAYERNORM);
        const op_t *d2 = mid ? nullptr : w->delta2.as<op_t>();
        float *r32 = w->resid.as<float>(); op_t *r16 = w->resid16.as<op_t>();
        const float *lw = Wf + w_off, *lb = Wf + b_off;
        const int wr = mid ? 0 : 1;
        if (last) {
            float *fo = w->final_out.as<float>(); op_t *eo = w->d_enc_bf16.as<op_t>();
            if (!resid16) launch_add_layernorm<float, float, float>(c, r32, r32, w->delta.as<op_t>(), d2, 1, lw, lb, M, d, fo, 1e-5f, eo);
            else if (first_layer) launch_add_layernorm<float, float, op_t>(c, r32, r16, w->delta.as<op_t>(), d2, 1, lw, lb, M, d, fo, 1e-5f, eo);
            else launch_add_layernorm<float, op_t, op_t>(c, r16, r16, w->delta.as<op_t>(), d2, 1, lw, lb, M, d, fo, 1e-5f, eo);
        } else {
            op_t *lo = w->ln_out.as<op_t>();
            if (!resid16) launch_add_layernorm<op_t, float, float>(c, r32, r32, w->delta.as<op_t>(), d2, wr, lw, lb, M, d, lo, 1e-5f, nullptr);
            else if (first_layer) launch_add_layernorm<op_t, float, op_t>(c, r32, r16, w->delta.as<op_t>(), d2, wr, lw, lb, M, d, lo, 1e-5f, nullptr);
            else launch_add_layernorm<op_t, op_t, op_t>(c, r16, r16, w->delta.as<op_t>(), d2, wr, lw, lb, M, d, lo, 1e-5f, nullptr);
        }
    };
    for (int l = 0; l < L; l++) {
        const WhisperState::Layer &ly = w->layers[(size_t)l];
        if (!flat || l == 0) {
            KernelTimer kt(c, PCE_K_LAYERNORM);
            launch_layernorm<op_t>(c, w->resid.as<float>(), Wf + ly.ln1_w, Wf + ly.ln1_b, M, d, w->ln_out.as<op_t>(), 1e-5f, nullptr, resid16 ? 1 : 0);
        }
        const bool done = flat && launch_gemm_flat<FEPI_SPLIT>(c, w->ln_out.as<op_t>(), Wb + ly.qkv_w, Wf + ly.qkv_b, w->qkv.as<op_t>(), (int)M, 3 * d, d, 2 * d,
                                                                W_CTX, AT_SP, PCE_K_GEMM_FLAT_QKV, w->vt.as<op_t>(), 2 * d);
        if (flat && !done) return pce_fail(c, PCE_E_LIMIT, "Q | K | V projection does not fit the 256 x 256 kernel");
        if (!done)
            launch_gemm<EPI_QKV>(c, w->ln_out.as<op_t>(), d, 0, Wb + ly.qkv_w, (int)M, 3 * d, d, Wf + ly.qkv_b, w->qkv.as<op_t>(), 2 * d, 0, 1,
                                 reinterpret_cast<const float *>(w->vt.as<op_t>()), W_CTX, 2 * d, AT_SP);
        {
            AttnArgs a{};
            a.q = w->qkv.as<op_t>(); a.q_ld = 2 * d; a.k = w->qkv.as<op_t>() + d; a.k_ld = 2 * d;
            a.vt = w->vt.as<op_t>(); a.vt_clip = (int64_t)d * AT_SP; a.vt_sp = AT_SP;
            a.q_row0 = a.k_row0 = w->enc_tab.as<int>(); a.q_len = a.k_len = w->enc_tab.as<int>() + n;
            a.out = w->attn.as<op_t>(); a.out_ld = d; a.causal = 0;
            launch_attention(c, dim3((unsigned)div_up(W_CTX, AT_QB), (unsigned)H, (unsigned)n), a, 4.0 * W_CTX * (double)W_CTX * d * n);
        }
        if (flat) {
            if (!launch_gemm_flat<FEPI_BF16>(c, w->attn.as<op_t>(), Wb + ly.out_w, Wf + ly.out_b, w->delta.as<op_t>(), (int)M, d, d, d, 1, 0, PCE_K_GEMM_FLAT_OUT))
                return pce_fail(c, PCE_E_LIMIT, "attention projection does not fit the 256 x 256 kernel");
            add_ln(ly.ln2_w, ly.ln2_b, true, false, l == 0);
            if (!launch_gemm_flat<FEPI_GELU>(c, w->ln_out.as<op_t>(), Wb + ly.m1_w, Wf + ly.m1_b, w->hidden.as<op_t>(), (int)M, 4 * d, d, 4 * d, 1, 0, PCE_K_GEMM_FLAT_FC1) ||
                !launch_gemm_flat<FEPI_BF16>(c, w->hidden.as<op_t>(), Wb + ly.m2_w, Wf + ly.m2_b, w->delta2.as<op_t>(), (int)M, d, 4 * d, d, 1, 0, PCE_K_GEMM_FLAT_FC2))
                return pce_fail(c, PCE_E_LIMIT, "MLP does not fit the 256 x 256 kernel");
            if (l + 1 < L) add_ln(w->layers[(size_t)l + 1].ln1_w, w->layers[(size_t)l + 1].ln1_b, false, false, l == 0);
            else add_ln(w->lnp_w, w->lnp_b, false, true, l == 0);
            continue;
        }
        launch_gemm<EPI_RESID_F32>(c, w->attn.as<op_t>(), d, 0, Wb + ly.out_w, (int)M, d, d, Wf + ly.out_b, w->resid.as<float>(), d, 0, 1);
        {
            KernelTimer kt(c, PCE_K_LAYERNORM);
            launch_layernorm<op_t>(c, w->resid.as<float>(), Wf + ly.ln2_w, Wf + ly.ln2_b, M, d, w->ln_out.as<op_t>());
        }
        launch_gemm<EPI_GELU_BF16>(c, w->ln_out.as<op_t>(), d, 0, Wb + ly.m1_w, (int)M, 4 * d, d, Wf + ly.m1_b, w->hidden.as<op_t>(), 4 * d, 0, 1);
        launch_gemm<EPI_RESID_F32>(c, w->hidden.as<op_t>(), 4 * d, 0, Wb + ly.m2_w, (int)M, d, 4 * d, Wf + ly.m2_b, w->resid.as<float>(), d, 0, 1);
    }
    if (!flat) {
        KernelTimer kt(c, PCE_K_LAYERNORM);
        launch_layernorm<float>(c, w->resid.as<float>(), Wf + w->lnp_w, Wf + w->lnp_b, M, d, w->final_out.as<float>());
    }
    PCE_HIP(c, hipGetLastError());
    w->n_clips_enc = n; w->g_xkv_clips = -1; w->g_cache_len = -1; w->g_keys_n = 0; w->enc_bf16_clips = flat ? n : -1;
    return PCE_OK;
}

static void project_cross_kv(pce_ctx *c, const op_t *enc, int Ma, int d, const op_t *W, const float *bias, op_t *xk, op_t *xvt)
{
    if (launch_gemm_flat<FEPI_SPLIT>(c, enc, W, bias, xk, Ma, 2 * d, d, d, W_CTX, AT_SP, PCE_K_GEMM_FLAT_XKV, xvt, d)) return;
    launch_gemm<EPI_QKV>(c, enc, d, 0, W, Ma, 2 * d, d, bias, xk, d, 0, 1, reinterpret_cast<const float *>(xvt), W_CTX, d, AT_SP);
}

static __global__ void k_selftest_vt(const op_t *__restrict__ v, int k_len, int hd, int sp, int64_t n, op_t *__restrict__ vt)
{
    const int64_t i = (int64_t)blockIdx.x * blockDim.x + threadIdx.x;
    if (i >= n) return;
    const int col = (int)(i % hd); const int64_t r = i / hd; const int t = (int)(r % k_len); const int64_t clip = r / k_len;
    vt[(clip * hd + col) * sp + t] = v[i];
}

int pce_selftest_attention(pce_ctx *c, const uint16_t *q, const uint16_t *k, const uint16_t *v, int32_t clips, int32_t heads, int32_t q_len,
                           int32_t k_len, int32_t causal, int32_t mode, uint16_t *out, int32_t *fell_back)
{
    if (!c || !q || !k || !v || !out || clips <= 0 || heads <= 0 || q_len <= 0 || k_len <= 0 || mode < 0 || mode > 1) return PCE_E_INVALID;
    PCE_HIP(c, hipSetDevice(c->device));
    const int hd = heads * 64, sp = div_up(k_len, 64) * 64;
    const size_t nq = (size_t)clips * q_len * hd, nk = (size_t)clips * k_len * hd, nvt = (size_t)clips * hd * sp;
    DevBuf dq, dk, dv, dvt, dout, dtab, dcnt;
    PCE_HIP(c, dq.reserve(nq * 2 + 64)); PCE_HIP(c, dk.reserve(nk * 2 + 64)); PCE_HIP(c, dv.reserve(nk * 2 + 64)); PCE_HIP(c, dvt.reserve(nvt * 2 + 128));
    PCE_HIP(c, dout.reserve(nq * 2 + 64)); PCE_HIP(c, dtab.reserve(sizeof(int) * 4 * (size_t)clips)); PCE_HIP(c, dcnt.reserve(sizeof(int)));
    std::vector<int> tab((size_t)4 * clips);
    for (int i = 0; i < clips; i++) { tab[(size_t)i] = i * q_len; tab[(size_t)clips + i] = q_len; tab[(size_t)2 * clips + i] = i * k_len; tab[(size_t)3 * clips + i] = k_len; }
    PCE_HIP(c, hipMemcpyAsync(dq.p, q, nq * 2, hipMemcpyHostToDevice, c->stream));
    PCE_HIP(c, hipMemcpyAsync(dk.p, k, nk * 2, hipMemcpyHostToDevice, c->stream));
    PCE_HIP(c, hipMemcpyAsync(dv.p, v, nk * 2, hipMemcpyHostToDevice, c->stream));
    PCE_HIP(c, hipMemcpyAsync(dtab.p, tab.data(), sizeof(int) * tab.size(), hipMemcpyHostToDevice, c->stream));
    PCE_HIP(c, hipMemsetAsync(dvt.p, 0, nvt * 2 + 128, c->stream));
    PCE_HIP(c, hipMemsetAsync(dout.p, 0, nq * 2, c->stream));
    PCE_HIP(c, hipMemsetAsync(dcnt.p, 0, sizeof(int), c->stream));
    hipLaunchKernelGGL(k_selftest_vt, dim3((unsigned)div_up((int64_t)nk, 256)), dim3(256), 0, c->stream, dv.as<op_t>(), k_len, hd, sp, (int64_t)nk, dvt.as<op_t>());
    AttnArgs a{};
    a.q = dq.as<op_t>(); a.q_ld = hd; a.k = dk.as<op_t>(); a.k_ld = hd; a.vt = dvt.as<op_t>(); a.vt_clip = (int64_t)hd * sp; a.vt_sp = sp;
    a.q_row0 = dtab.as<int>(); a.q_len = a.q_row0 + clips; a.k_row0 = a.q_row0 + 2 * clips; a.k_len = a.q_row0 + 3 * clips;
    a.out = dout.as<op_t>(); a.out_ld = hd; a.causal = causal; a.fell_back = dcnt.as<int>();
    const dim3 grid((unsigned)div_up(q_len, AT_QB), (unsigned)heads, (unsigned)clips);
    hipLaunchKernelGGL(k_attention_lean16<false>, grid, dim3(256), 0, c->stream, a, mode);
    PCE_HIP(c, hipGetLastError());
    int cnt = 0;
    PCE_HIP(c, hipMemcpyAsync(out, dout.p, nq * 2, hipMemcpyDeviceToHost, c->stream));
    PCE_HIP(c, hipMemcpyAsync(&cnt, dcnt.p, sizeof(int), hipMemcpyDeviceToHost, c->stream));
    PCE_HIP(c, hipStreamSynchronize(c->stream));
    if (fell_back) *fell_back = cnt;
    return PCE_OK;
}

int pce_selftest_xattn(pce_ctx *c, const float *resid, const float *ln_w, const float *ln_b, const uint16_t *wq, const float *bq, const uint16_t *wk,
                       const uint16_t *wv, const float *bv, const uint16_t *E, const int32_t *k_len, int32_t n, int32_t k_cap, int32_t d, int32_t heads,
                       int32_t workgroups_per_clip, uint16_t *out)
{
    if (!c || !resid || !ln_w || !ln_b || !wq || !bq || !wk || !wv || !bv || !E || !k_len || !out || n <= 0 || k_cap <= 0) return PCE_E_INVALID;
    if (!xa_has_form(d, heads))
        return pce_fail(c, PCE_E_INVALID, "selftest xattn: d = %d with %d heads is not a width the encoder-output form is built for", d, heads);
    if (!(workgroups_per_clip == 0 || workgroups_per_clip == 1 || workgroups_per_clip == 2 || workgroups_per_clip == 4)) return PCE_E_INVALID;
    for (int i = 0; i < n; i++) if (k_len[i] <= 0 || k_len[i] > k_cap) return pce_fail(c, PCE_E_INVALID, "selftest xattn: clip %d has %d frames of %d", i, k_len[i], k_cap);
    PCE_HIP(c, hipSetDevice(c->device));
    { const int rc = lds_optins(c, ws_of(c)); if (rc) return rc; }
    const size_t dd = (size_t)d * d, ne = (size_t)n * k_cap * d;
    DevBuf dres, dlw, dlb, dwq, dbq, dwk, dwkT, dwv, dbv, dE, dkl, dqp, dup, dml, dout;
    PCE_HIP(c, dres.reserve(sizeof(float) * (size_t)n * d)); PCE_HIP(c, dlw.reserve(sizeof(float) * d)); PCE_HIP(c, dlb.reserve(sizeof(float) * d));
    PCE_HIP(c, dwq.reserve(2 * dd)); PCE_HIP(c, dbq.reserve(sizeof(float) * d)); PCE_HIP(c, dwk.reserve(2 * dd)); PCE_HIP(c, dwkT.reserve(2 * dd));
    PCE_HIP(c, dwv.reserve(2 * dd)); PCE_HIP(c, dbv.reserve(sizeof(float) * d)); PCE_HIP(c, dE.reserve(2 * ne + 4096)); PCE_HIP(c, dkl.reserve(sizeof(int) * (size_t)n));
    const size_t R = (size_t)xa_rows(heads);
    PCE_HIP(c, dqp.reserve(2 * 2 * (size_t)n * R * d + 256)); PCE_HIP(c, dup.reserve(sizeof(float) * (size_t)n * XA_MAX_SPLIT * R * d + 256));
    PCE_HIP(c, dml.reserve(sizeof(float) * (size_t)n * XA_MAX_SPLIT * R * 2 + 256)); PCE_HIP(c, dout.reserve(2 * (size_t)n * d + 64));
    struct Up { void *dst; const void *src; size_t bytes; } ups[] = {
        {dres.p, resid, sizeof(float) * (size_t)n * d}, {dlw.p, ln_w, sizeof(float) * d}, {dlb.p, ln_b, sizeof(float) * d}, {dwq.p, wq, 2 * dd}, {dbq.p, bq, sizeof(float) * d},
        {dwk.p, wk, 2 * dd}, {dwv.p, wv, 2 * dd}, {dbv.p, bv, sizeof(float) * d}, {dE.p, E, 2 * ne}, {dkl.p, k_len, sizeof(int) * (size_t)n}};
    for (const Up &u : ups) PCE_HIP(c, hipMemcpyAsync(u.dst, u.src, u.bytes, hipMemcpyHostToDevice, c->stream));
    PCE_HIP(c, hipMemsetAsync(dqp.p, 0, dqp.cap, c->stream)); PCE_HIP(c, hipMemsetAsync(dout.p, 0, dout.cap, c->stream));
    hipLaunchKernelGGL(k_transpose_sq, dim3((unsigned)(d / 32), (unsigned)(d / 32)), dim3(256), 0, c->stream, dwk.as<op_t>(), dwkT.as<op_t>(), d);
    XaArgs a{};
    a.E = dE.as<op_t>(); a.e_clip = (int64_t)k_cap * d; a.e_ld = d; a.k_len = dkl.as<int>(); a.skip = nullptr;
    a.u_part = dup.as<float>(); a.ml_part = dml.as<float>(); a.heads = heads; a.nsplit = xa_split(n, workgroups_per_clip); a.rows = (int)R;
    XaLayer y{};
    y.resid = dres.as<float>(); y.ln_w = dlw.as<float>(); y.ln_b = dlb.as<float>(); y.wq = dwq.as<op_t>(); y.bq = dbq.as<float>(); y.wkT = dwkT.as<op_t>();
    y.wv = dwv.as<op_t>(); y.bv = dbv.as<float>(); y.qp_hi = dqp.as<op_t>(); y.qp_lo = y.qp_hi + (size_t)n * R * d; y.out = dout.as<op_t>(); y.out_ld = d;
    xattn_launch(c, d, n, a, y);
    PCE_HIP(c, hipGetLastError());
    PCE_HIP(c, hipMemcpyAsync(out, dout.p, 2 * (size_t)n * d, hipMemcpyDeviceToHost, c->stream));
    PCE_HIP(c, hipStreamSynchronize(c->stream));
    return PCE_OK;
}

int pce_selftest_gemm(pce_ctx *c, const uint16_t *A, const uint16_t *B, const float *bias, int32_t M, int32_t N, int32_t K, int32_t epilogue,
                      int32_t rows_per_clip, int32_t vt_sp, uint16_t *out)
{
    if (!c || !A || !B || !out || M <= 0 || N <= 0 || K <= 0) return PCE_E_INVALID;
    PCE_HIP(c, hipSetDevice(c->device));
    { const int rc = lds_optins(c, ws_of(c)); if (rc) return rc; }
    if (epilogue >= 16 && epilogue <= 19) {
        const bool f32 = epilogue == 19;
        DevBuf tA, tB, tC, tb;
        PCE_HIP(c, tA.reserve((size_t)M * K * 2 + 4096)); PCE_HIP(c, tB.reserve((size_t)(N + 128) * K * 2 + 4096)); PCE_HIP(c, tC.reserve((size_t)M * N * 4 + 4096));
        PCE_HIP(c, tb.reserve((size_t)(N + 128) * 4));
        PCE_HIP(c, hipMemsetAsync(tB.p, 0, (size_t)(N + 128) * K * 2, c->stream));
        PCE_HIP(c, hipMemcpyAsync(tA.p, A, (size_t)M * K * 2, hipMemcpyHostToDevice, c->stream));
        PCE_HIP(c, hipMemcpyAsync(tB.p, B, (size_t)N * K * 2, hipMemcpyHostToDevice, c->stream));
        PCE_HIP(c, hipMemsetAsync(tb.p, 0, (size_t)(N + 128) * 4, c->stream));
        if (bias) PCE_HIP(c, hipMemcpyAsync(tb.p, bias, (size_t)N * 4, hipMemcpyHostToDevice, c->stream));
        PCE_HIP(c, hipMemsetAsync(tC.p, 0, (size_t)M * N * 4, c->stream));
        if (N % 128) return pce_fail(c, PCE_E_INVALID, "selftest gemm (tiled): N must be a multiple of 128");
        c->gemm_few_rows = true;
        struct Off { pce_ctx *c; ~Off() { c->gemm_few_rows = false; } } off{c};
        if (epilogue == 16) launch_gemm<EPI_BF16>(c, tA.as<op_t>(), K, 0, tB.as<op_t>(), M, N, K, tb.as<float>(), tC.p, N, 0, 1);
        else if (epilogue == 17) launch_gemm<EPI_GELU_BF16>(c, tA.as<op_t>(), K, 0, tB.as<op_t>(), M, N, K, tb.as<float>(), tC.p, N, 0, 1);
        else if (epilogue == 19) launch_gemm<EPI_RESID_F32>(c, tA.as<op_t>(), K, 0, tB.as<op_t>(), M, N, K, tb.as<float>(), tC.p, N, 0, 1);
        else return pce_fail(c, PCE_E_INVALID, "selftest gemm: epilogue 18 does not exist");
        PCE_HIP(c, hipGetLastError());
        PCE_HIP(c, hipMemcpyAsync(out, tC.p, (size_t)M * N * (f32 ? 4 : 2), hipMemcpyDeviceToHost, c->stream));
        PCE_HIP(c, hipStreamSynchronize(c->stream));
        pce_profile_collect(c);
        return PCE_OK;
    }
    const size_t n_out = epilogue == 2 ? (size_t)(M / rows_per_clip) * N * vt_sp
                         : epilogue >= 256 ? (size_t)M * epilogue + (size_t)(M / rows_per_clip) * (N - epilogue) * vt_sp : (size_t)M * N;
    DevBuf dA, dB, dC, dbias;
    PCE_HIP(c, dA.reserve((size_t)M * K * 2)); PCE_HIP(c, dB.reserve((size_t)N * K * 2)); PCE_HIP(c, dC.reserve(n_out * 2)); PCE_HIP(c, dbias.reserve((size_t)N * 4));
    PCE_HIP(c, hipMemcpyAsync(dA.p, A, (size_t)M * K * 2, hipMemcpyHostToDevice, c->stream));
    PCE_HIP(c, hipMemcpyAsync(dB.p, B, (size_t)N * K * 2, hipMemcpyHostToDevice, c->stream));
    if (bias) PCE_HIP(c, hipMemcpyAsync(dbias.p, bias, (size_t)N * 4, hipMemcpyHostToDevice, c->stream));
    PCE_HIP(c, hipMemsetAsync(dC.p, 0, n_out * 2, c->stream));
    bool ok = false;
    const float *bp = bias ? dbias.as<float>() : nullptr;
    if (epilogue == 0) ok = launch_gemm_flat<FEPI_BF16>(c, dA.as<op_t>(), dB.as<op_t>(), bp, dC.as<op_t>(), M, N, K, N);
    else if (epilogue == 1) ok = launch_gemm_flat<FEPI_GELU>(c, dA.as<op_t>(), dB.as<op_t>(), bp, dC.as<op_t>(), M, N, K, N);
    else if (epilogue == 2) ok = launch_gemm_flat<FEPI_VT>(c, dA.as<op_t>(), dB.as<op_t>(), bp, dC.as<op_t>(), M, N, K, 0, rows_per_clip, vt_sp);
    else if (epilogue >= 256 && epilogue % 256 == 0 && epilogue < N)
        ok = launch_gemm_flat<FEPI_SPLIT>(c, dA.as<op_t>(), dB.as<op_t>(), bp, dC.as<op_t>(), M, N, K, epilogue, rows_per_clip, vt_sp, PCE_K_GEMM_FLAT,
                                          dC.as<op_t>() + (size_t)M * epilogue, epilogue);
    int rc = PCE_OK;
    if (!ok) rc = pce_fail(c, PCE_E_LIMIT, "shape not handled by the 256 x 256 kernel (N %% 256, K %% 64)");
    else {
        hipError_t e = hipGetLastError();
        if (e == hipSuccess) e = hipMemcpyAsync(out, dC.p, n_out * 2, hipMemcpyDeviceToHost, c->stream);
        if (e == hipSuccess) e = hipStreamSynchronize(c->stream);
        if (e != hipSuccess) rc = pce_fail(c, PCE_E_DEVICE, "selftest gemm: %s", hipGetErrorString(e));
    }
    (void)hipStreamSynchronize(c->stream);
    pce_profile_collect(c);
    return rc;
}

int pce_selftest_gemm_tiled(pce_ctx *c, int32_t kernel, int32_t epilogue, const uint16_t *A, int64_t a_len, int64_t lda, int64_t a_batch, int32_t batch,
                            const uint16_t *B, const float *bias, int32_t M, int32_t N, int32_t K, void *C, int64_t c_len, int64_t ldc, int64_t c_batch,
                            const float *pos, int32_t pos_T, int32_t v_col0, int32_t rows_per_clip, int32_t vt_sp, uint16_t *vt, int64_t vt_len,
                            int32_t *kernel_used)
{
    if (!c || !A || !B || !C || M <= 0 || N <= 0 || K <= 0 || batch <= 0 || kernel < GK_AUTO || kernel > GK_128_DEEP || epilogue < EPI_BF16 || epilogue > EPI_F32)
        return PCE_E_INVALID;
    const bool f32 = epilogue == EPI_GELU_POS_F32 || epilogue == EPI_RESID_F32 || epilogue == EPI_F32, qkv = epilogue == EPI_QKV;
    const int64_t nc = qkv ? v_col0 : N;
    if (lda < 1 || lda % 8 || a_batch < 0 || a_batch % 8 || ldc < nc || ldc % 8 || c_batch < 0 || c_batch % 8)
        return pce_fail(c, PCE_E_INVALID, "selftest gemm (tiled): lda, a_batch, ldc, c_batch must be multiples of 8 (16-byte rows), ldc >= the output columns");
    if ((int64_t)(batch - 1) * a_batch + (int64_t)(M - 1) * lda + K > a_len)
        return pce_fail(c, PCE_E_INVALID, "selftest gemm (tiled): A holds %lld elements, the shape reads beyond them", (long long)a_len);
    if (nc > 0 && (int64_t)(batch - 1) * c_batch + (int64_t)(M - 1) * ldc + nc > c_len)
        return pce_fail(c, PCE_E_INVALID, "selftest gemm (tiled): C holds %lld elements, the shape writes beyond them", (long long)c_len);
    if (epilogue == EPI_GELU_POS_F32 && (!pos || pos_T < 1)) return pce_fail(c, PCE_E_INVALID, "selftest gemm (tiled): GELU_POS_F32 needs pos [pos_T][N]");
    int64_t n_vt = 0;
    if (qkv) {
        const int S = rows_per_clip;
        if (!vt || batch != 1 || v_col0 < 0 || v_col0 >= N || (N - v_col0) % 64 || S < 4 || S % 4 || vt_sp < S || vt_sp % 4)
            return pce_fail(c, PCE_E_INVALID, "selftest gemm (tiled): QKV needs vt, batch 1, 0 <= v_col0 < N, rows_per_clip %% 4 == 0, rows_per_clip <= vt_sp, vt_sp %% 4 == 0");
        n_vt = (int64_t)div_up(M, S) * (N - v_col0) * vt_sp;
        if (n_vt > vt_len) return pce_fail(c, PCE_E_INVALID, "selftest gemm (tiled): vt holds %lld elements, the V image needs %lld", (long long)vt_len, (long long)n_vt);
    }
    const GemmShape s{M, N, K, lda, batch, qkv ? v_col0 : 0};
    const int kind = epilogue == EPI_BF16 ? selftest_gemm_kind<EPI_BF16>(c, kernel, s) : epilogue == EPI_GELU_BF16 ? selftest_gemm_kind<EPI_GELU_BF16>(c, kernel, s)
                     : epilogue == EPI_GELU_POS_F32 ? selftest_gemm_kind<EPI_GELU_POS_F32>(c, kernel, s) : epilogue == EPI_RESID_F32 ? selftest_gemm_kind<EPI_RESID_F32>(c, kernel, s)
                     : epilogue == EPI_QKV ? selftest_gemm_kind<EPI_QKV>(c, kernel, s) : selftest_gemm_kind<EPI_F32>(c, kernel, s);
    if (kind < 0)
        return pce_fail(c, PCE_E_LIMIT, "selftest gemm (tiled): kernel %d does not compute epilogue %d at M %d x N %d x K %d (lda %lld, batch %d, v_col0 %d)",
                        kernel, epilogue, M, N, K, (long long)lda, batch, v_col0);
    if (kernel_used) *kernel_used = kind;
    PCE_HIP(c, hipSetDevice(c->device));
    { const int rc = lds_optins(c, ws_of(c)); if (rc) return rc; }
    const size_t esz = f32 ? 4 : 2;
    DevBuf dA, dB, dbias, dC, dpos, dvt;
    PCE_HIP(c, dA.reserve(2 * (size_t)a_len)); PCE_HIP(c, dB.reserve(2 * (size_t)N * K)); PCE_HIP(c, dC.reserve(esz * (size_t)c_len + 16));
    PCE_HIP(c, hipMemcpyAsync(dA.p, A, 2 * (size_t)a_len, hipMemcpyHostToDevice, c->stream));
    PCE_HIP(c, hipMemcpyAsync(dB.p, B, 2 * (size_t)N * K, hipMemcpyHostToDevice, c->stream));
    PCE_HIP(c, hipMemcpyAsync(dC.p, C, esz * (size_t)c_len, hipMemcpyHostToDevice, c->stream));
    if (bias) { PCE_HIP(c, dbias.reserve(sizeof(float) * N)); PCE_HIP(c, hipMemcpyAsync(dbias.p, bias, sizeof(float) * N, hipMemcpyHostToDevice, c->stream)); }
    if (epilogue == EPI_GELU_POS_F32) {
        PCE_HIP(c, dpos.reserve(sizeof(float) * (size_t)pos_T * N));
        PCE_HIP(c, hipMemcpyAsync(dpos.p, pos, sizeof(float) * (size_t)pos_T * N, hipMemcpyHostToDevice, c->stream));
    }
    if (qkv) { PCE_HIP(c, dvt.reserve(2 * (size_t)vt_len)); PCE_HIP(c, hipMemcpyAsync(dvt.p, vt, 2 * (size_t)vt_len, hipMemcpyHostToDevice, c->stream)); }
    const op_t *a = dA.as<op_t>(), *b = dB.as<op_t>();
    const float *bp = bias ? dbias.as<float>() : nullptr;
    switch (epilogue) {
    case EPI_BF16: launch_gemm_kernel<EPI_BF16>(c, kind, a, lda, a_batch, b, M, N, K, bp, dC.p, ldc, c_batch, batch, nullptr, 1, 0, 0); break;
    case EPI_GELU_BF16: launch_gemm_kernel<EPI_GELU_BF16>(c, kind, a, lda, a_batch, b, M, N, K, bp, dC.p, ldc, c_batch, batch, nullptr, 1, 0, 0); break;
    case EPI_GELU_POS_F32: launch_gemm_kernel<EPI_GELU_POS_F32>(c, kind, a, lda, a_batch, b, M, N, K, bp, dC.p, ldc, c_batch, batch, dpos.as<float>(), pos_T, 0, 0); break;
    case EPI_RESID_F32: launch_gemm_kernel<EPI_RESID_F32>(c, kind, a, lda, a_batch, b, M, N, K, bp, dC.p, ldc, c_batch, batch, nullptr, 1, 0, 0); break;
    case EPI_QKV:
        launch_gemm_kernel<EPI_QKV>(c, kind, a, lda, a_batch, b, M, N, K, bp, dC.p, ldc, c_batch, batch, reinterpret_cast<const float *>(dvt.as<op_t>()),
                                    rows_per_clip, v_col0, vt_sp);
        break;
    default: launch_gemm_kernel<EPI_F32>(c, kind, a, lda, a_batch, b, M, N, K, bp, dC.p, ldc, c_batch, batch, nullptr, 1, 0, 0); break;
    }
    PCE_HIP(c, hipGetLastError());
    PCE_HIP(c, hipMemcpyAsync(C, dC.p, esz * (size_t)c_len, hipMemcpyDeviceToHost, c->stream));
    if (qkv) PCE_HIP(c, hipMemcpyAsync(vt, dvt.p, 2 * (size_t)vt_len, hipMemcpyDeviceToHost, c->stream));
    PCE_HIP(c, hipStreamSynchronize(c->stream));
    pce_profile_collect(c);
    return PCE_OK;
}

int pce_selftest_layernorm(pce_ctx *c, int32_t form, int32_t rows, int32_t d, const void *x, const uint16_t *delta, const uint16_t *delta2, const float *w,
                           const float *b, float eps, int32_t flags, void *out, void *resid_out, uint16_t *out_copy)
{
    if (!c || !x || !w || !b || !out || rows <= 0 || form < 0 || form > 7) return PCE_E_INVALID;
    if (d < 4 || d % 4 || d > LN_D_MAX) return pce_fail(c, PCE_E_LIMIT, "selftest layernorm: d = %d (need d %% 4 == 0, d <= %d)", d, LN_D_MAX);
    PCE_HIP(c, hipSetDevice(c->device));
    const size_t n = (size_t)rows * d;
    if (form <= 1) {
        const bool in_place = flags & 2;
        if (in_place && !resid_out) return PCE_E_INVALID;
        DevBuf dx, dw, db, dout;
        PCE_HIP(c, dx.reserve(sizeof(float) * n)); PCE_HIP(c, dw.reserve(sizeof(float) * d)); PCE_HIP(c, db.reserve(sizeof(float) * d));
        PCE_HIP(c, dout.reserve((form ? 2 : 4) * n));
        PCE_HIP(c, hipMemcpyAsync(dx.p, x, sizeof(float) * n, hipMemcpyHostToDevice, c->stream));
// ... 898 lines not shown
```

prosody-control-french-tts_amd/engine.py:

```python
from __future__ import annotations

import ctypes as C
import os
import subprocess

import numpy as np

_HERE = os.path.dirname(os.path.abspath(__file__))
_LIB_PATH = os.path.join(_HERE, "libpce.so")


class PceError(RuntimeError):
    pass


def native_library_path() -> str:
    return os.environ.get("PCE_LIBRARY") or _LIB_PATH


def build_native(force: bool = False) -> str:
    csrc = os.path.join(_HERE, "csrc")
    if force:
        subprocess.check_call(["make", "-C", csrc, "clean"], stdout=subprocess.DEVNULL)
    subprocess.check_call(["make", "-C", csrc, "-j4"], stdout=subprocess.DEVNULL)
    if not os.path.exists(_LIB_PATH):
        raise PceError("build did not produce libpce.so")
    return _LIB_PATH


class Slice(C.Structure):
    _fields_ = [("clip", C.c_int32), ("flags", C.c_int32), ("begin", C.c_int64), ("end", C.c_int64), ("x1", C.c_double)]


class Energy(C.Structure):
    _fields_ = [("n", C.c_int64), ("sum_sq", C.c_int64), ("sum_sq_wrap16", C.c_int64), ("n_loud", C.c_int64),
                ("peak_abs", C.c_int32), ("reserved", C.c_int32)]


class PitchParams(C.Structure):
    _fields_ = [("time_step", C.c_double), ("pitch_floor", C.c_double), ("periods_per_window", C.c_double),
                ("max_candidates", C.c_int32), ("reserved", C.c_int32), ("silence_threshold", C.c_double),
                ("voicing_threshold", C.c_double), ("octave_cost", C.c_double), ("octave_jump_cost", C.c_double),
                ("voiced_unvoiced_cost", C.c_double), ("pitch_ceiling", C.c_double)]

    @classmethod
    def praat(cls, pitch_floor=75.0, pitch_ceiling=600.0, time_step=0.0):
        return cls(time_step or 0.0, float(pitch_floor), 3.0, 15, 0, 0.03, 0.45, 0.01, 0.35, 0.14, float(pitch_ceiling))


class PitchSummary(C.Structure):
    _fields_ = [("n_frames", C.c_int64), ("n_voiced", C.c_int64), ("median_f0", C.c_double), ("mean_log_f0", C.c_double),
                ("t1", C.c_double), ("status", C.c_int32), ("reserved", C.c_int32)]


class WhisperDims(C.Structure):
    _fields_ = [("n_mels", C.c_int32), ("n_ctx", C.c_int32), ("n_state", C.c_int32), ("n_head", C.c_int32), ("n_layer", C.c_int32)]


class WhisperTextDims(C.Structure):
    _fields_ = [("n_vocab", C.c_int32), ("n_text_ctx", C.c_int32), ("n_state", C.c_int32), ("n_head", C.c_int32), ("n_layer", C.c_int32)]


class WhisperDecodeRules(C.Structure):
    _fields_ = [("eot", C.c_int32), ("timestamp_begin", C.c_int32), ("max_initial_timestamp_index", C.c_int32), ("reserved", C.c_int32)]


class WhisperDecodeOpts(C.Structure):
    _fields_ = [("sample_begin", C.c_void_p), ("sample_begin_all", C.c_int32), ("temperature", C.c_float), ("seed_lo", C.c_uint32),
                ("seed_hi", C.c_uint32), ("probe_token", C.c_int32), ("flags", C.c_int32)]


class BertDims(C.Structure):
    _fields_ = [("n_vocab", C.c_int32), ("n_pos", C.c_int32), ("n_type", C.c_int32), ("n_state", C.c_int32), ("n_head", C.c_int32),
                ("n_layer", C.c_int32), ("n_labels", C.c_int32)]


SLICE_DTYPE = np.dtype([("clip", "<i4"), ("flags", "<i4"), ("begin", "<i8"), ("end", "<i8"), ("x1", "<f8")])
ENERGY_DTYPE = np.dtype([("n", "<i8"), ("sum_sq", "<i8"), ("sum_sq_wrap16", "<i8"), ("n_loud", "<i8"),
                         ("peak_abs", "<i4"), ("reserved", "<i4")])
SUMMARY_DTYPE = np.dtype([("n_frames", "<i8"), ("n_voiced", "<i8"), ("median_f0", "<f8"), ("mean_log_f0", "<f8"),
                          ("t1", "<f8"), ("status", "<i4"), ("reserved", "<i4")])
assert SLICE_DTYPE.itemsize == C.sizeof(Slice) and ENERGY_DTYPE.itemsize == C.sizeof(Energy)
assert SUMMARY_DTYPE.itemsize == C.sizeof(PitchSummary)

SLICE_OK, SLICE_TOO_SHORT, SLICE_EMPTY = 0, 1, 2
DTW_OK, DTW_EMPTY, DTW_NO_PATH = 0, 1, 2
DTW_SERIES_ROWS, DTW_SERIES_COLS = 1024, 2048

KERNEL_IDS = ["k_energy", "k_lufs_pass1", "k_lufs_scan", "k_lufs_pass2", "k_lufs_gate",
              "k_pitch_refine", "k_pitch_frames", "k_pitch_path", "k_pitch_median", "k_pitch_delta", "k_stft_max", "k_stft_db", "k_logmel_frames", "whisper_encoder", "k_resample", "k_dtw", "whisper_align", "k_nw", "k_stft_norm", "k_frame_energy", "bert_forward", "k_pyin_frames", "k_pyin_viterbi", "whisper_decode_step",
              "k_gemm_bf16", "k_gemm_wide", "k_attention", "k_layernorm", "k_gemm_flat",
              "k_add_layernorm", "k_stft_raw", "k_logmel_norm", "k_attention_lean",
              "k_gemm_flat:qkv", "k_gemm_flat:out", "k_gemm_flat:fc1", "k_gemm_flat:fc2", "k_gemm_flat:xkv",
              "whisper_decode_loop", "k_cross_attn1", "k_gemm_skinny", "k_levenshtein", "k_dtw_series", "k_dtw_series_trace"]

EXPORTS = ["pce_create", "pce_destroy", "pce_last_error", "pce_sync", "pce_api_version", "pce_api_minor", "pce_device_info",
           "pce_upload_pcm_s16", "pce_bind_pcm_s16_device", "pce_num_clips",
           "pce_energy_run", "pce_energy_fetch", "pce_lufs_set_meter_rate", "pce_lufs_run", "pce_lufs_fetch",
           "pce_frame_energy_run", "pce_frame_energy_shape", "pce_frame_energy_fetch", "pce_pyin_run", "pce_pyin_shape", "pce_pyin_fetch",
           "pce_pitch_plan", "pce_pitch_run", "pce_pitch_set_refine", "pce_pitch_fetch",
           "pce_stft_db_run", "pce_stft_db_shape", "pce_stft_db_fetch", "pce_stft_db_device",
           "pce_resample_run", "pce_download_pcm_s16",
           "pce_dtw", "pce_dtw_series", "pce_nw_align", "pce_levenshtein", "pce_whisper_decoder_load", "pce_whisper_align_run", "pce_whisper_align_shape", "pce_whisper_align_fetch", "pce_whisper_align_paths_enqueue", "pce_whisper_align_paths_wait", "pce_whisper_sample_keys", "pce_whisper_decode_step", "pce_whisper_decode_step_ex", "pce_whisper_decode_loop", "pce_whisper_set_operands", "pce_whisper_get_operands", "pce_selftest_xattn", "pce_selftest_gemm_tiled", "pce_selftest_layernorm",
           "pce_logmel_run", "pce_logmel_run_at", "pce_logmel_fetch", "pce_whisper_load", "pce_whisper_encode_run", "pce_selftest_gemm", "pce_selftest_attention", "pce_whisper_encode_fetch",
           "pce_stats_enqueue", "pce_stats_wait", "pce_bert_load", "pce_bert_run", "pce_bert_fetch",
           "pce_profile_enable", "pce_profile_reset", "pce_profile_get", "pce_profile_get_work", "pce_kernel_name"]


def load_library() -> C.CDLL:
    path = native_library_path()
    if not os.path.exists(path):
        raise PceError(f"{path} is missing: run __graft_entry__.build() (hipcc --offload-arch=gfx950); "
                       "this engine has no CPU fallback")
    lib = C.CDLL(path)
    vp, i32, i64 = C.c_void_p, C.c_int32, C.c_int64
    lib.pce_create.argtypes = [C.c_int, vp, C.c_char_p, C.c_size_t]; lib.pce_create.restype = vp
    lib.pce_destroy.argtypes = [vp]; lib.pce_destroy.restype = None
    lib.pce_last_error.argtypes = [vp]; lib.pce_last_error.restype = C.c_char_p
    lib.pce_sync.argtypes = [vp]
    lib.pce_api_version.argtypes = []
    lib.pce_api_minor.argtypes = []
    lib.pce_device_info.argtypes = [vp, C.c_char_p, C.c_size_t, C.POINTER(i32), C.POINTER(i64)]
    lib.pce_upload_pcm_s16.argtypes = [vp, vp, vp, i32, i32]
    lib.pce_bind_pcm_s16_device.argtypes = [vp, vp, vp, i32, i32]
    lib.pce_num_clips.argtypes = [vp]
    lib.pce_energy_run.argtypes = [vp, vp, i32, i32]
    lib.pce_energy_fetch.argtypes = [vp, vp]
    lib.pce_lufs_set_meter_rate.argtypes = [vp, i32]
    lib.pce_pitch_set_refine.argtypes = [vp, i32]
    lib.pce_lufs_run.argtypes = [vp, vp, i32]
    lib.pce_frame_energy_run.argtypes = [vp, i32, i32, i32]
    lib.pce_pyin_run.argtypes = [vp, vp, vp, i64]
    lib.pce_pyin_shape.argtypes = [vp, i32, C.POINTER(i64)]
    lib.pce_pyin_fetch.argtypes = [vp, i32, vp, vp, C.POINTER(i32)]
    lib.pce_frame_energy_shape.argtypes = [vp, i32, C.POINTER(i64)]
    lib.pce_frame_energy_fetch.argtypes = [vp, i32, vp, vp]
    lib.pce_lufs_fetch.argtypes = [vp, vp, vp]
    lib.pce_pitch_plan.argtypes = [vp, C.POINTER(PitchParams), vp, i32, vp, vp]
    lib.pce_pitch_run.argtypes = [vp, C.POINTER(PitchParams), vp, i32]
    lib.pce_pitch_fetch.argtypes = [vp, vp, vp, vp]
    lib.pce_stats_enqueue.argtypes = [vp, i32]
    lib.pce_nw_align.argtypes = [vp, vp, vp, vp, vp, i32, i32, i32, i32, vp, vp, vp]
    lib.pce_levenshtein.argtypes = [vp, vp, vp, vp, vp, i32, vp]
    lib.pce_stats_wait.argtypes = [vp, i32, vp, vp, vp, vp]
    lib.pce_stft_db_run.argtypes = [vp, i32, i32]
    lib.pce_stft_db_shape.argtypes = [vp, i32, C.POINTER(i32), C.POINTER(i32)]
    lib.pce_stft_db_fetch.argtypes = [vp, i32, vp]
    lib.pce_stft_db_device.argtypes = [vp, C.POINTER(vp), C.POINTER(i64)]
    lib.pce_resample_run.argtypes = [vp, i32, i32, vp, i32, i64]
    lib.pce_download_pcm_s16.argtypes = [vp, vp, vp, C.POINTER(i32)]
    lib.pce_dtw.argtypes = [vp, vp, i32, i32, i32, vp, vp, vp]
    lib.pce_dtw_series.argtypes = [vp, vp, vp, vp, vp, vp, vp, i32, vp, vp, vp, vp, vp]
    lib.pce_whisper_decoder_load.argtypes = [vp, C.POINTER(WhisperTextDims), vp, i64]
    lib.pce_whisper_align_run.argtypes = [vp, vp, vp, vp, i32, vp, i32, C.c_float]
    lib.pce_whisper_align_shape.argtypes = [vp, i32, C.POINTER(i32), C.POINTER(i32)]
    lib.pce_whisper_decode_step.argtypes = [vp, vp, vp, i32, C.POINTER(WhisperDecodeRules), vp, vp, vp]
    lib.pce_whisper_decode_step_ex.argtypes = [vp, vp, vp, C.POINTER(WhisperDecodeRules), vp, C.POINTER(WhisperDecodeOpts), vp, vp, vp]
    lib.pce_whisper_set_operands.argtypes = [vp, i32]
    lib.pce_whisper_get_operands.argtypes = [vp]
    lib.pce_whisper_decode_loop.argtypes = [vp, vp, vp, C.POINTER(WhisperDecodeRules), vp, C.POINTER(WhisperDecodeOpts), i32, i32, vp, vp, vp, vp]
    lib.pce_whisper_align_fetch.argtypes = [vp, i32, vp, vp, C.POINTER(i32), vp]
    lib.pce_whisper_align_paths_enqueue.argtypes = [vp, i32, C.POINTER(i32), C.POINTER(i32)]
    lib.pce_whisper_align_paths_wait.argtypes = [vp, i32, vp, vp, vp]
    lib.pce_whisper_sample_keys.argtypes = [vp, vp, i32]
    lib.pce_bert_load.argtypes = [vp, C.POINTER(BertDims), vp, i64]
    lib.pce_bert_run.argtypes = [vp, vp, vp, i32]
    lib.pce_bert_fetch.argtypes = [vp, i32, vp, vp]
    lib.pce_logmel_run.argtypes = [vp, i32]
    lib.pce_logmel_run_at.argtypes = [vp, i32, vp]
    lib.pce_logmel_fetch.argtypes = [vp, i32, vp]
    lib.pce_whisper_load.argtypes = [vp, C.POINTER(WhisperDims), vp, i64]
    lib.pce_whisper_encode_run.argtypes = [vp]
    lib.pce_selftest_gemm.argtypes = [vp, vp, vp, vp, i32, i32, i32, i32, i32, i32, vp]
    lib.pce_selftest_attention.argtypes = [vp, vp, vp, vp, i32, i32, i32, i32, i32, i32, vp, vp]
    lib.pce_selftest_xattn.argtypes = [vp] * 11 + [i32] * 5 + [vp]
    lib.pce_selftest_gemm_tiled.argtypes = [vp, i32, i32, vp, i64, i64, i64, i32, vp, vp, i32, i32, i32, vp, i64, i64, i64, vp, i32, i32, i32, i32, vp, i64, vp]
    lib.pce_selftest_layernorm.argtypes = [vp, i32, i32, i32, vp, vp, vp, vp, vp, C.c_float, i32, vp, vp, vp]
    lib.pce_whisper_encode_fetch.argtypes = [vp, i32, vp]
    lib.pce_profile_enable.argtypes = [vp, C.c_int]
    lib.pce_profile_reset.argtypes = [vp]
    lib.pce_profile_get.argtypes = [vp, C.c_int, C.POINTER(C.c_double), C.POINTER(i64)]
    lib.pce_profile_get_work.argtypes = [vp, C.c_int, C.POINTER(C.c_double)]
    lib.pce_kernel_name.argtypes = [C.c_int]; lib.pce_kernel_name.restype = C.c_char_p
    for name in EXPORTS:
        fn = getattr(lib, name)
        if fn.restype is C.c_int and name not in ("pce_create",):
            fn.restype = C.c_int
    return lib


def make_slices(clips, begins, ends, x1=None) -> np.ndarray:
    n = len(clips)
    s = np.zeros(n, dtype=SLICE_DTYPE)
    s["clip"] = clips; s["begin"] = begins; s["end"] = ends
    if x1 is not None:
        s["x1"] = x1
    return s


class ProsodyEngine:

    def __init__(self, device: int = 0, stream: int | None = None):
        self._lib = load_library()
        err = C.create_string_buffer(512)
        self._ctx = self._lib.pce_create(int(device), C.c_void_p(stream) if stream else None, err, len(err))
        if not self._ctx:
            raise PceError(f"pce_create failed: {err.value.decode(errors='replace')}")
        self.device = int(device)
        self.rate = 0
        self.clip_lengths = np.zeros(0, dtype=np.int64)
        self._keep = []

    def close(self):
        if getattr(self, "_ctx", None):
            self._lib.pce_destroy(self._ctx)
            self._ctx = None

    def __del__(self):
        try:
            self.close()
        except Exception:
            pass

    def __enter__(self):
        return self

    def __exit__(self, *a):
        self.close()

    def _check(self, rc: int):
        if rc != 0:
            raise PceError(f"libpce status {rc}: {self._lib.pce_last_error(self._ctx).decode(errors='replace')}")

    def sync(self):
        self._check(self._lib.pce_sync(self._ctx))

    def device_info(self):
        name = C.create_string_buffer(256); cus = C.c_int32(); hbm = C.c_int64()
        self._check(self._lib.pce_device_info(self._ctx, name, len(name), C.byref(cus), C.byref(hbm)))
        return {"name": name.value.decode(), "compute_units": cus.value, "hbm_bytes": hbm.value}

    def upload(self, clips, rate: int):
        clips = [np.ascontiguousarray(c, dtype=np.int16).reshape(-1) for c in clips]
        lens = np.array([len(c) for c in clips], dtype=np.int64)
        offsets = np.zeros(len(clips) + 1, dtype=np.int64)
        np.cumsum(lens, out=offsets[1:])
        pcm = np.concatenate(clips) if clips else np.zeros(0, dtype=np.int16)
        if pcm.size == 0:
            pcm = np.zeros(1, dtype=np.int16)
        self._check(self._lib.pce_upload_pcm_s16(self._ctx, pcm.ctypes.data, offsets.ctypes.data, len(clips), int(rate)))
        self.rate = int(rate); self.clip_lengths = lens; self.offsets = offsets
        return self

    def bind_device(self, device_ptr: int, offsets, rate: int, keepalive=None):
        offsets = np.ascontiguousarray(offsets, dtype=np.int64)
        self._check(self._lib.pce_bind_pcm_s16_device(self._ctx, C.c_void_p(device_ptr), offsets.ctypes.data,
# ... 108 lines not shown
        taps = np.ascontiguousarray(taps, dtype=np.float64)
        self._check(self._lib.pce_resample_run(self._ctx, up, down, taps.ctypes.data, len(taps), n_pre_remove))
        off = np.zeros(len(self.clip_lengths) + 1, dtype=np.int64); rate = C.c_int32()
        self._check(self._lib.pce_download_pcm_s16(self._ctx, None, off.ctypes.data, C.byref(rate)))
        self.rate, self.offsets, self.clip_lengths = rate.value, off, np.diff(off)
        return self

    def download(self):
        pcm = np.zeros(max(int(self.offsets[-1]), 1), dtype=np.int16)
        self._check(self._lib.pce_download_pcm_s16(self._ctx, pcm.ctypes.data, None, None))
        return [pcm[self.offsets[i]:self.offsets[i + 1]].copy() for i in range(len(self.clip_lengths))]

    def logmel_run(self, n_mels: int = 80):
        self._n_mels = int(n_mels)
        self._check(self._lib.pce_logmel_run(self._ctx, int(n_mels)))

    def logmel_run_at(self, n_mels: int, start_frames):
        sf = np.ascontiguousarray(start_frames, dtype=np.int64)
        self._check(self._lib.pce_logmel_run_at(self._ctx, int(n_mels), sf.ctypes.data))
        self._n_mels = int(n_mels)

    def logmel_fetch(self, clip: int) -> np.ndarray:
        out = np.zeros((self._n_mels, 3000), dtype=np.float32)
        self._check(self._lib.pce_logmel_fetch(self._ctx, int(clip), out.ctypes.data))
        return out

    def whisper_set_operands(self, kind: str):
        code = {"bf16": 0, "fp16": 1, "fp16-resid16": 2}[str(kind).lower()]
        self._check(self._lib.pce_whisper_set_operands(self._ctx, code))

    @property
    def whisper_operands(self) -> str:
        code = self._lib.pce_whisper_get_operands(self._ctx)
        if code < 0:
            self._check(code)
        return {0: "bf16", 1: "fp16", 2: "fp16-resid16"}.get(code, f"mode-{code}")

    def _op_dtype(self):
        import torch
        return torch.bfloat16 if self.whisper_operands == "bf16" else torch.float16

    def whisper_load(self, dims: dict, weights: np.ndarray):
        w = np.ascontiguousarray(weights, dtype=np.float32)
        self._wdims = WhisperDims(dims["n_mels"], dims["n_ctx"], dims["n_state"], dims["n_head"], dims["n_layer"])
        self._check(self._lib.pce_whisper_load(self._ctx, C.byref(self._wdims), w.ctypes.data, w.size))

    def whisper_encode_run(self):
        self._check(self._lib.pce_whisper_encode_run(self._ctx))
        self._n_encoded = len(self.clip_lengths)

    def whisper_num_encoded(self) -> int:
        return getattr(self, "_n_encoded", 0)

    def whisper_sample_keys(self, keys=None):
        if keys is None or len(keys) == 0:
            self._check(self._lib.pce_whisper_sample_keys(self._ctx, None, 0)); return
        k = np.ascontiguousarray(np.asarray(keys, dtype=np.int64) & 0x7FFFFFFF, dtype=np.int32)
        self._check(self._lib.pce_whisper_sample_keys(self._ctx, k.ctypes.data, int(k.size)))

    def selftest_gemm(self, A, B, bias=None, epilogue: int = 0, rows_per_clip: int = 1, vt_sp: int = 0):
        import torch
        a = torch.from_numpy(np.ascontiguousarray(A, dtype=np.float32)).to(self._op_dtype()).contiguous()
        b = torch.from_numpy(np.ascontiguousarray(B, dtype=np.float32)).to(self._op_dtype()).contiguous()
        M, K = a.shape; N = b.shape[0]
        if 16 <= epilogue <= 19:
            f32 = epilogue == 19
            outb = np.zeros(M * N, dtype=np.float32) if f32 else torch.zeros(M * N, dtype=self._op_dtype())
            bvv = None if bias is None else np.ascontiguousarray(bias, dtype=np.float32)
            self._check(self._lib.pce_selftest_gemm(self._ctx, a.view(torch.int16).numpy().ctypes.data, b.view(torch.int16).numpy().ctypes.data,
                                                    bvv.ctypes.data if bvv is not None else None, M, N, K, int(epilogue), 1, 0,
                                                    outb.ctypes.data if f32 else outb.view(torch.int16).numpy().ctypes.data))
            return outb.reshape(M, N) if f32 else outb.float().numpy().reshape(M, N)
        split = epilogue if epilogue >= 256 else 0
        n_out = (M // rows_per_clip) * N * vt_sp if epilogue == 2 else M * split + (M // rows_per_clip) * (N - split) * vt_sp if split else M * N
        out = torch.zeros(n_out, dtype=self._op_dtype())
        bv = None if bias is None else np.ascontiguousarray(bias, dtype=np.float32)
        self._check(self._lib.pce_selftest_gemm(self._ctx, a.view(torch.int16).numpy().ctypes.data, b.view(torch.int16).numpy().ctypes.data,
                                                bv.ctypes.data if bv is not None else None, M, N, K, int(epilogue), int(rows_per_clip), int(vt_sp),
                                                out.view(torch.int16).numpy().ctypes.data))
        res = out.float().numpy()
        if split:
            return res[:M * split].reshape(M, split), res[M * split:].reshape(M // rows_per_clip, N - split, vt_sp)
        return res.reshape(M // rows_per_clip, N, vt_sp) if epilogue == 2 else res.reshape(M, N)

    def selftest_attention(self, q, k, v, causal: bool = False, mode: int = 0):
        import torch
        tq, tk, tv = (torch.from_numpy(np.ascontiguousarray(x, dtype=np.float32)).to(self._op_dtype()).contiguous() for x in (q, k, v))
        clips, q_len, hd = tq.shape
        k_len = tk.shape[1]
        assert hd % 64 == 0 and tk.shape == tv.shape == (clips, k_len, hd)
        out = torch.zeros_like(tq)
        fb = C.c_int32(0)
        self._check(self._lib.pce_selftest_attention(self._ctx, tq.view(torch.int16).numpy().ctypes.data, tk.view(torch.int16).numpy().ctypes.data,
                                                     tv.view(torch.int16).numpy().ctypes.data, clips, hd // 64, q_len, k_len, int(bool(causal)), int(mode),
                                                     out.view(torch.int16).numpy().ctypes.data, C.addressof(fb)))
        return out.float().numpy(), int(fb.value)

    def selftest_xattn(self, resid, ln_w, ln_b, wq, bq, wk, wv, bv, E, k_len, heads: int, workgroups_per_clip: int = 0):
        import torch
        dt = self._op_dtype()
        r16 = lambda x: torch.from_numpy(np.ascontiguousarray(x, dtype=np.float32)).to(dt).contiguous()
        tq, tk, tv, tE = r16(wq), r16(wk), r16(wv), r16(E)
        n, k_cap, d = tE.shape
        f32 = lambda x: np.ascontiguousarray(x, dtype=np.float32)
        res, lw, lb, vq, vv = f32(resid), f32(ln_w), f32(ln_b), f32(bq), f32(bv)
        kl = np.ascontiguousarray(k_len, dtype=np.int32)
        out = torch.zeros((n, d), dtype=dt)
        ptr = lambda t: t.view(torch.int16).numpy().ctypes.data
        self._check(self._lib.pce_selftest_xattn(self._ctx, res.ctypes.data, lw.ctypes.data, lb.ctypes.data, ptr(tq), vq.ctypes.data, ptr(tk), ptr(tv), vv.ctypes.data,
                                                 ptr(tE), kl.ctypes.data, int(n), int(k_cap), int(d), int(heads), int(workgroups_per_clip), ptr(out)))
        return out.float().numpy(), tq.float().numpy(), tk.float().numpy(), tv.float().numpy(), tE.float().numpy()

    def selftest_gemm_tiled(self, epilogue: int, A, B, bias, M: int, N: int, K: int, C, lda: int, ldc: int, kernel: int = 0, a_batch: int = 0,
                            batch: int = 1, c_batch: int = 0, pos=None, v_col0: int = 0, rows_per_clip: int = 0, vt=None, vt_sp: int = 0) -> int:
        def arr(x, dt):
            assert isinstance(x, np.ndarray) and x.dtype == dt and x.flags["C_CONTIGUOUS"], (None if x is None else x.dtype, dt)
            return x
        f32 = epilogue in (2, 3, 5)
        A, B, C = arr(A, np.uint16), arr(B, np.uint16), arr(C, np.float32 if f32 else np.uint16)
        assert B.size == N * K
        bv = None if bias is None else np.ascontiguousarray(bias, dtype=np.float32)
        assert bv is None or bv.size == N
        pv = None if pos is None else np.ascontiguousarray(pos, dtype=np.float32)
        assert pv is None or pv.size % N == 0
        if vt is not None:
            arr(vt, np.uint16)
        used = np.zeros(1, dtype=np.int32)
        self._check(self._lib.pce_selftest_gemm_tiled(self._ctx, int(kernel), int(epilogue), A.ctypes.data, A.size, int(lda), int(a_batch), int(batch),
                                                      B.ctypes.data, None if bv is None else bv.ctypes.data, int(M), int(N), int(K), C.ctypes.data, C.size,
                                                      int(ldc), int(c_batch), None if pv is None else pv.ctypes.data, 0 if pv is None else pv.size // N,
                                                      int(v_col0), int(rows_per_clip), int(vt_sp), None if vt is None else vt.ctypes.data,
                                                      0 if vt is None else vt.size, used.ctypes.data))
        return int(used[0])

    def selftest_layernorm(self, form: int, x, w, b, eps: float = 1e-5, flags: int = 0, delta=None, delta2=None, want_copy: bool = False):
        x = np.ascontiguousarray(x)
        rows, d = x.shape
        o, st = (form - 2) // 3, (form - 2) % 3
        assert x.dtype == (np.uint16 if form >= 2 and st == 2 else np.float32)
        out = np.zeros((rows, d), dtype=np.uint16 if form == 1 or (form >= 2 and o == 1) else np.float32)
        if form <= 1:
            resid = np.zeros((rows, d), dtype=np.float32) if flags & 2 else None
        else:
            resid = np.zeros((rows, d), dtype=np.float32 if st == 0 else np.uint16)
        cp = np.zeros((rows, d), dtype=np.uint16) if want_copy else None
        f = lambda v: np.ascontiguousarray(v, dtype=np.float32)
        u = lambda v: None if v is None else np.ascontiguousarray(v, dtype=np.uint16)
        w, b, delta, delta2 = f(w), f(b), u(delta), u(delta2)
        ptr = lambda v: None if v is None else v.ctypes.data
        self._check(self._lib.pce_selftest_layernorm(self._ctx, int(form), rows, d, x.ctypes.data, ptr(delta), ptr(delta2), w.ctypes.data, b.ctypes.data,
                                                     float(eps), int(flags), out.ctypes.data, ptr(resid), ptr(cp)))
        return out, resid, cp

    def whisper_encode_fetch(self, clip: int) -> np.ndarray:
        out = np.zeros((1500, self._wdims.n_state), dtype=np.float32)
        self._check(self._lib.pce_whisper_encode_fetch(self._ctx, int(clip), out.ctypes.data))
        return out

    def whisper_decoder_load(self, dims: dict, weights: np.ndarray):
        w = np.ascontiguousarray(weights, dtype=np.float32)
        self._tdims = WhisperTextDims(dims["n_vocab"], dims["n_text_ctx"], dims["n_state"], dims["n_head"], dims["n_layer"])
        self._check(self._lib.pce_whisper_decoder_load(self._ctx, C.byref(self._tdims), w.ctypes.data, w.size))

    def whisper_align_run(self, token_lists, num_frames, sot_len: int, head_mask=None, medfilt_width: int = 7, qk_scale: float = 1.0):
        toks = np.concatenate([np.asarray(t, dtype=np.int32) for t in token_lists]).astype(np.int32)
        off = np.zeros(len(token_lists) + 1, dtype=np.int32); np.cumsum([len(t) for t in token_lists], out=off[1:])
# ... 251 lines not shown
```

Baseline: 20470.

## Fuse residual add into flat GEMM epilogue and layernorm on fp16 residual

Adds a residual epilogue to the 256x256 flat GEMM that loads the fp16 residual tile, adds the bias-applied output, and writes back in place. Under resid16, the attention-out and FC2 projections now accumulate directly into the fp16 residual, and the following add+layernorm is replaced by a plain layernorm that reads fp16. This removes the delta/delta2 buffers and their round trip through memory. The costs are 16 extra 128-bit registers per thread for the residual tile and an extra global load in the GEMM epilogue. The first layer's layernorm also writes the fp16 residual copy, and a selftest entry point is added.

```diff
diff --git a/include/pce.h b/include/pce.h
--- a/include/pce.h
+++ b/include/pce.h
@@ -11,7 +11,7 @@
 #pragma GCC visibility push(default)
 
 #define PCE_API_VERSION 1
-#define PCE_API_MINOR 6
+#define PCE_API_MINOR 7
 
 typedef struct pce_ctx pce_ctx;
 
@@ -131,6 +131,7 @@
 int pce_whisper_encode_run(pce_ctx *ctx);
 int pce_selftest_gemm(pce_ctx *ctx, const uint16_t *A, const uint16_t *B, const float *bias, int32_t M, int32_t N, int32_t K, int32_t epilogue,
                       int32_t rows_per_clip, int32_t vt_sp, uint16_t *out);
+int pce_selftest_gemm_resid(pce_ctx *ctx, const uint16_t *A, const uint16_t *B, const float *bias, int32_t M, int32_t N, int32_t K, uint16_t *C);
 int pce_selftest_attention(pce_ctx *ctx, const uint16_t *q, const uint16_t *k, const uint16_t *v, int32_t clips, int32_t heads, int32_t q_len,
                            int32_t k_len, int32_t causal, int32_t mode, uint16_t *out, int32_t *fell_back);
 int pce_selftest_xattn(pce_ctx *ctx, const float *resid, const float *ln_w, const float *ln_b, const uint16_t *wq, const float *bq, const uint16_t *wk,
diff --git a/prosody-control-french-tts_amd/csrc/pce_gemm256.inc b/prosody-control-french-tts_amd/csrc/pce_gemm256.inc
--- a/prosody-control-french-tts_amd/csrc/pce_gemm256.inc
+++ b/prosody-control-french-tts_amd/csrc/pce_gemm256.inc
@@ -4,7 +4,7 @@
 constexpr bool F_PINGPONG = true;
 constexpr int F_HALF = 128 * F_K;
 constexpr int F_RING_BYTES = 8 * F_HALF * 2;
-enum { FEPI_BF16 = 0, FEPI_GELU = 1, FEPI_VT = 2, FEPI_SPLIT = 3 };
+enum { FEPI_BF16 = 0, FEPI_GELU = 1, FEPI_VT = 2, FEPI_SPLIT = 3, FEPI_RESID = 4 };
 
 __device__ __forceinline__ int f_swz(int row, int chunk) { return chunk ^ ((row >> 1) & 7); }
 __device__ __forceinline__ int f_perm32(int p) { return ((p >> 2) & 3) * 8 + (p >> 4) * 4 + (p & 3); }
@@ -149,6 +149,19 @@
     const __amdgpu_buffer_rsrc_t rsC = __builtin_amdgcn_make_buffer_rsrc(P.C, 0, HAS_RM ? (int)((unsigned)M * (unsigned)P.ldc * 2u) : 0, 0x00020000);
     const __amdgpu_buffer_rsrc_t rsV = __builtin_amdgcn_make_buffer_rsrc(vt_ptr, 0, HAS_VT ? (int)((unsigned)(M / P.S) * (unsigned)Nv * (unsigned)P.vt_sp * 2u) : 0, 0x00020000);
     const int voffC = (fr * P.ldc + fq * 8) * 2, voffV = (fr * P.vt_sp + fq * 8) * 2;
+    u32x4 xres[16];
+    auto load_resid = [&](int m0, int n0) {
+#pragma unroll
+        for (int hB = 0; hB < 2; hB++)
+#pragma unroll
+            for (int hA = 0; hA < 2; hA++)
+#pragma unroll
+                for (int i = 0; i < 4; i++) {
+                    const unsigned soff = ((unsigned)(m0 + hA * 128 + wr * 64 + i * 16) * (unsigned)P.ldc + (unsigned)(n0 + hB * 128 + wc * 32)) * 2u;
+                    xres[(hB * 2 + hA) * 4 + i] = __builtin_amdgcn_raw_buffer_load_b128(rsC, voffC, (int)soff, 0);
+                }
+        __builtin_amdgcn_sched_barrier(0);
+    };
     auto store_rm = [&](int m0, int n0) {
 #pragma unroll
         for (int hB = 0; hB < 2; hB++) {
@@ -166,6 +179,11 @@
                     if (EPI == FEPI_GELU) gelu_exact8(t);
 #pragma unroll
                     for (int e = 0; e < 8; e++) o[e] = (op_t)t[e];
+                    if constexpr (EPI == FEPI_RESID) {
+                        const opx8 x = __builtin_bit_cast(opx8, xres[(hB * 2 + hA) * 4 + i]);
+#pragma unroll
+                        for (int e = 0; e < 8; e++) o[e] = (op_t)((float)x[e] + (float)o[e]);
+                    }
                     const unsigned soff = ((unsigned)(m0 + hA * 128 + wr * 64 + i * 16) * (unsigned)P.ldc + (unsigned)(n0 + hB * 128 + wc * 32)) * 2u;
                     __builtin_amdgcn_raw_buffer_store_b128(__builtin_bit_cast(u32x4, o), rsC, voffC, (int)soff, F_STORE_AUX);
                     __builtin_amdgcn_sched_barrier(0);
@@ -333,6 +351,7 @@
             else kstep(first && it > 0);
             pc1 = pc2; it1 = it2; kt1 = kt2; advance(pc2, it2, kt2);
             if (last) {
+                if constexpr (EPI == FEPI_RESID) load_resid(c_m0, c_n0);
                 if (F_PINGPONG && wr == 0) __builtin_amdgcn_s_barrier();
                 if constexpr (SPLIT) { if (cur_vt) store_vtT(c_m0, c_n0); else store_rm(c_m0, c_n0); }
                 else if constexpr (EPI == FEPI_VT) store_vt(c_m0, c_n0, c_n0);
diff --git a/prosody-control-french-tts_amd/csrc/pce_whisper_dispatch.hip b/prosody-control-french-tts_amd/csrc/pce_whisper_dispatch.hip
--- a/prosody-control-french-tts_amd/csrc/pce_whisper_dispatch.hip
+++ b/prosody-control-french-tts_amd/csrc/pce_whisper_dispatch.hip
@@ -11,6 +11,7 @@
 PCE_BOTH(int, pce_whisper_encode_fetch, (pce_ctx *, int32_t, float *))
 PCE_BOTH(int, pce_selftest_attention, (pce_ctx *, const uint16_t *, const uint16_t *, const uint16_t *, int32_t, int32_t, int32_t, int32_t, int32_t, int32_t, uint16_t *, int32_t *))
 PCE_BOTH(int, pce_selftest_gemm, (pce_ctx *, const uint16_t *, const uint16_t *, const float *, int32_t, int32_t, int32_t, int32_t, int32_t, int32_t, uint16_t *))
+PCE_BOTH(int, pce_selftest_gemm_resid, (pce_ctx *, const uint16_t *, const uint16_t *, const float *, int32_t, int32_t, int32_t, uint16_t *))
 PCE_BOTH(int, pce_selftest_xattn, (pce_ctx *, const float *, const float *, const float *, const uint16_t *, const float *, const uint16_t *, const uint16_t *, const float *, const uint16_t *, const int32_t *, int32_t, int32_t, int32_t, int32_t, int32_t, uint16_t *))
 PCE_BOTH(int, pce_selftest_gemm_tiled, (pce_ctx *, int32_t, int32_t, const uint16_t *, int64_t, int64_t, int64_t, int32_t, const uint16_t *, const float *, int32_t, int32_t,
                                          int32_t, void *, int64_t, int64_t, int64_t, const float *, int32_t, int32_t, int32_t, int32_t, uint16_t *, int64_t, int32_t *))
@@ -62,6 +63,10 @@
                       int32_t vt_sp, uint16_t *out)
 {
     return PCE_FWD(pce_selftest_gemm, c, A, B, bias, M, N, K, epilogue, rows_per_clip, vt_sp, out);
+}
+int pce_selftest_gemm_resid(pce_ctx *c, const uint16_t *A, const uint16_t *B, const float *bias, int32_t M, int32_t N, int32_t K, uint16_t *C)
+{
+    return PCE_FWD(pce_selftest_gemm_resid, c, A, B, bias, M, N, K, C);
 }
 int pce_selftest_xattn(pce_ctx *c, const float *resid, const float *ln_w, const float *ln_b, const uint16_t *wq, const float *bq, const uint16_t *wk, const uint16_t *wv,
                        const float *bv, const uint16_t *E, const int32_t *k_len, int32_t n, int32_t k_cap, int32_t d, int32_t heads, int32_t workgroups_per_clip, uint16_t *out)
diff --git a/prosody-control-french-tts_amd/csrc/pce_whisper_impl.inc b/prosody-control-french-tts_amd/csrc/pce_whisper_impl.inc
--- a/prosody-control-french-tts_amd/csrc/pce_whisper_impl.inc
+++ b/prosody-control-french-tts_amd/csrc/pce_whisper_impl.inc
@@ -11,6 +11,7 @@
 #define pce_whisper_encode_fetch PCE_WFN(pce_whisper_encode_fetch)
 #define pce_selftest_attention PCE_WFN(pce_selftest_attention)
 #define pce_selftest_gemm PCE_WFN(pce_selftest_gemm)
+#define pce_selftest_gemm_resid PCE_WFN(pce_selftest_gemm_resid)
 #define pce_whisper_decoder_load PCE_WFN(pce_whisper_decoder_load)
 #define pce_whisper_align_run PCE_WFN(pce_whisper_align_run)
 #define pce_whisper_align_fetch PCE_WFN(pce_whisper_align_fetch)
@@ -679,22 +680,32 @@
 }
 
 constexpr int LN_D_MAX = 2048;
-template <class OUT, int NV = 5>
-__global__ __launch_bounds__(256) void k_layernorm(const float *x, const float *__restrict__ w, const float *__restrict__ b,
-                                                  int64_t rows, int d, OUT *__restrict__ out, float eps = 1e-5f, float *out2 = nullptr, int round_in16 = 0)
+template <class OUT, int NV = 5, class IN = float>
+__global__ __launch_bounds__(256) void k_layernorm(const IN *x, const float *__restrict__ w, const float *__restrict__ b,
+                                                  int64_t rows, int d, OUT *__restrict__ out, float eps = 1e-5f, float *out2 = nullptr, int round_in16 = 0,
+                                                  op_t *__restrict__ x16 = nullptr, op_t *__restrict__ out16 = nullptr)
 {
     const int64_t row = (int64_t)blockIdx.x * 4 + (threadIdx.x >> 6);
     const int lane = threadIdx.x & 63;
     if (row >= rows) return;
-    const float4 *xr = reinterpret_cast<const float4 *>(x + row * d);
+    typedef __attribute__((ext_vector_type(4))) op_t opx4;
     const int nv = d >> 2;
     float4 v[NV];
     float s = 0.f;
 #pragma unroll
     for (int i = 0; i < NV; i++) {
         const int idx = lane + 64 * i;
-        v[i] = idx < nv ? xr[idx] : make_float4(0.f, 0.f, 0.f, 0.f);
-        if (round_in16) v[i] = make_float4((float)(op_t)v[i].x, (float)(op_t)v[i].y, (float)(op_t)v[i].z, (float)(op_t)v[i].w);
+        if constexpr (std::is_same<IN, float>::value) {
+            v[i] = idx < nv ? reinterpret_cast<const float4 *>(x + row * d)[idx] : make_float4(0.f, 0.f, 0.f, 0.f);
+            if (round_in16) {
+                opx4 h; h[0] = (op_t)v[i].x; h[1] = (op_t)v[i].y; h[2] = (op_t)v[i].z; h[3] = (op_t)v[i].w;
+                v[i] = make_float4((float)h[0], (float)h[1], (float)h[2], (float)h[3]);
+                if (x16 && idx < nv) __builtin_nontemporal_store(h, reinterpret_cast<opx4 *>(x16 + row * d) + idx);
+            }
+        } else if (idx < nv) {
+            const opx4 h = __builtin_nontemporal_load(reinterpret_cast<const opx4 *>(x + row * d) + idx);
+            v[i] = make_float4((float)h[0], (float)h[1], (float)h[2], (float)h[3]);
+        } else v[i] = make_float4(0.f, 0.f, 0.f, 0.f);
         s += (v[i].x + v[i].y) + (v[i].z + v[i].w);
     }
     s = wave_allsum_f32(s);
@@ -718,6 +729,7 @@
                         y2 = (v[i].z - mean) * inv * ww.z + bb.z, y3 = (v[i].w - mean) * inv * ww.w + bb.w;
             ln_store4<OUT>(out + row * d + 4 * idx, y0, y1, y2, y3);
             if (out2) ln_store4<float>(out2 + row * d + 4 * idx, y0, y1, y2, y3);
+            if (out16) ln_store4<op_t>(out16 + row * d + 4 * idx, y0, y1, y2, y3);
         }
     }
 }
@@ -1809,11 +1821,18 @@
 
 template <class OUT>
 static void launch_layernorm(pce_ctx *c, const float *x, const float *w, const float *b, int64_t rows, int d, OUT *out, float eps = 1e-5f,
-                             float *out2 = nullptr, int round_in16 = 0)
+                             float *out2 = nullptr, int round_in16 = 0, op_t *x16 = nullptr)
 {
     const dim3 grid((unsigned)div_up(rows, 4)), block(256);
-    if (d <= 1280) hipLaunchKernelGGL((k_layernorm<OUT, 5>), grid, block, 0, c->stream, x, w, b, rows, d, out, eps, out2, round_in16);
-    else hipLaunchKernelGGL((k_layernorm<OUT, 8>), grid, block, 0, c->stream, x, w, b, rows, d, out, eps, out2, round_in16);
+    if (d <= 1280) hipLaunchKernelGGL((k_layernorm<OUT, 5>), grid, block, 0, c->stream, x, w, b, rows, d, out, eps, out2, round_in16, x16, (op_t *)nullptr);
+    else hipLaunchKernelGGL((k_layernorm<OUT, 8>), grid, block, 0, c->stream, x, w, b, rows, d, out, eps, out2, round_in16, x16, (op_t *)nullptr);
+}
+template <class OUT>
+static void launch_layernorm16(pce_ctx *c, const op_t *x, const float *w, const float *b, int64_t rows, int d, OUT *out, float eps, op_t *out16)
+{
+    const dim3 grid((unsigned)div_up(rows, 4)), block(256);
+    if (d <= 1280) hipLaunchKernelGGL((k_layernorm<OUT, 5, op_t>), grid, block, 0, c->stream, x, w, b, rows, d, out, eps, (float *)nullptr, 0, (op_t *)nullptr, out16);
+    else hipLaunchKernelGGL((k_layernorm<OUT, 8, op_t>), grid, block, 0, c->stream, x, w, b, rows, d, out, eps, (float *)nullptr, 0, (op_t *)nullptr, out16);
 }
 template <class OUT, class RIN, class ROUT>
 static void launch_add_layernorm(pce_ctx *c, const RIN *resid_in, ROUT *resid_out, const op_t *delta, const op_t *delta2, int write_resid, const float *w,
@@ -1893,6 +1912,7 @@
     PCE_HIP(c, hipFuncSetAttribute((const void *)k_gemm_flat<FEPI_GELU>, A, flat));
     PCE_HIP(c, hipFuncSetAttribute((const void *)k_gemm_flat<FEPI_VT>, A, flat));
     PCE_HIP(c, hipFuncSetAttribute((const void *)k_gemm_flat<FEPI_SPLIT>, A, flat));
+    PCE_HIP(c, hipFuncSetAttribute((const void *)k_gemm_flat<FEPI_RESID>, A, flat));
     PCE_HIP(c, hipFuncSetAttribute((const void *)k_gemm_skinny<EPI_BF16>, A, S_LDS));
     PCE_HIP(c, hipFuncSetAttribute((const void *)k_gemm_skinny<EPI_GELU_BF16>, A, S_LDS));
     PCE_HIP(c, hipFuncSetAttribute((const void *)k_gemm_skinny<EPI_RESID_F32>, A, S_LDS));
@@ -2171,35 +2191,30 @@
                                   Wf + w->c2_b, w->resid.as<float>(), d, (int64_t)W_CTX * d, n, w->pos.as<float>(), W_CTX);
     const bool flat = c->gemm_flat && d % F_T == 0 && gemm_flat_offsets_fit(M, 4 * d, 4 * d, 4 * d, 0, 0) &&
                       gemm_flat_offsets_fit(M, d, d, 0, W_CTX, AT_SP);
-    if (flat) {
-        PCE_HIP(c, w->delta.reserve(sizeof(op_t) * (size_t)M * d)); PCE_HIP(c, w->delta2.reserve(sizeof(op_t) * (size_t)M * d));
-        PCE_HIP(c, w->d_enc_bf16.reserve(sizeof(op_t) * (size_t)M * d + 4096));
-    }
     const bool resid16 = flat && c->resid16 && PCE_OP_INDEX == 1;
+    if (flat) PCE_HIP(c, w->d_enc_bf16.reserve(sizeof(op_t) * (size_t)M * d + 4096));
     if (resid16) PCE_HIP(c, w->resid16.reserve(sizeof(op_t) * (size_t)M * d));
-    auto add_ln = [&](size_t w_off, size_t b_off, bool mid, bool last, bool first_layer) {
+    else if (flat) { PCE_HIP(c, w->delta.reserve(sizeof(op_t) * (size_t)M * d)); PCE_HIP(c, w->delta2.reserve(sizeof(op_t) * (size_t)M * d)); }
+    auto add_ln = [&](size_t w_off, size_t b_off, bool mid, bool last) {
+        const float *lw = Wf + w_off, *lb = Wf + b_off;
+        if (resid16) {
+            KernelTimer kt(c, PCE_K_LAYERNORM);
+            if (last) launch_layernorm16<float>(c, w->resid16.as<op_t>(), lw, lb, M, d, w->final_out.as<float>(), 1e-5f, w->d_enc_bf16.as<op_t>());
+            else launch_layernorm16<op_t>(c, w->resid16.as<op_t>(), lw, lb, M, d, w->ln_out.as<op_t>(), 1e-5f, nullptr);
+            return;
+        }
         KernelTimer kt(c, PCE_K_ADD_LAYERNORM);
         const op_t *d2 = mid ? nullptr : w->delta2.as<op_t>();
-        float *r32 = w->resid.as<float>(); op_t *r16 = w->resid16.as<op_t>();
-        const float *lw = Wf + w_off, *lb = Wf + b_off;
-        const int wr = mid ? 0 : 1;
-        if (last) {
-            float *fo = w->final_out.as<float>(); op_t *eo = w->d_enc_bf16.as<op_t>();
-            if (!resid16) launch_add_layernorm<float, float, float>(c, r32, r32, w->delta.as<op_t>(), d2, 1, lw, lb, M, d, fo, 1e-5f, eo);
-            else if (first_layer) launch_add_layernorm<float, float, op_t>(c, r32, r16, w->delta.as<op_t>(), d2, 1, lw, lb, M, d, fo, 1e-5f, eo);
-            else launch_add_layernorm<float, op_t, op_t>(c, r16, r16, w->delta.as<op_t>(), d2, 1, lw, lb, M, d, fo, 1e-5f, eo);
-        } else {
-            op_t *lo = w->ln_out.as<op_t>();
-            if (!resid16) launch_add_layernorm<op_t, float, float>(c, r32, r32, w->delta.as<op_t>(), d2, wr, lw, lb, M, d, lo, 1e-5f, nullptr);
-            else if (first_layer) launch_add_layernorm<op_t, float, op_t>(c, r32, r16, w->delta.as<op_t>(), d2, wr, lw, lb, M, d, lo, 1e-5f, nullptr);
-            else launch_add_layernorm<op_t, op_t, op_t>(c, r16, r16, w->delta.as<op_t>(), d2, wr, lw, lb, M, d, lo, 1e-5f, nullptr);
-        }
+        float *r32 = w->resid.as<float>();
+        if (last) launch_add_layernorm<float, float, float>(c, r32, r32, w->delta.as<op_t>(), d2, 1, lw, lb, M, d, w->final_out.as<float>(), 1e-5f, w->d_enc_bf16.as<op_t>());
+        else launch_add_layernorm<op_t, float, float>(c, r32, r32, w->delta.as<op_t>(), d2, mid ? 0 : 1, lw, lb, M, d, w->ln_out.as<op_t>(), 1e-5f, nullptr);
     };
     for (int l = 0; l < L; l++) {
         const WhisperState::Layer &ly = w->layers[(size_t)l];
         if (!flat || l == 0) {
             KernelTimer kt(c, PCE_K_LAYERNORM);
-            launch_layernorm<op_t>(c, w->resid.as<float>(), Wf + ly.ln1_w, Wf + ly.ln1_b, M, d, w->ln_out.as<op_t>(), 1e-5f, nullptr, resid16 ? 1 : 0);
+            launch_layernorm<op_t>(c, w->resid.as<float>(), Wf + ly.ln1_w, Wf + ly.ln1_b, M, d, w->ln_out.as<op_t>(), 1e-5f, nullptr, resid16 ? 1 : 0,
+                                   resid16 ? w->resid16.as<op_t>() : nullptr);
         }
         const bool done = flat && launch_gemm_flat<FEPI_SPLIT>(c, w->ln_out.as<op_t>(), Wb + ly.qkv_w, Wf + ly.qkv_b, w->qkv.as<op_t>(), (int)M, 3 * d, d, 2 * d,
                                                                 W_CTX, AT_SP, PCE_K_GEMM_FLAT_QKV, w->vt.as<op_t>(), 2 * d);
@@ -2216,14 +2231,17 @@
             launch_attention(c, dim3((unsigned)div_up(W_CTX, AT_QB), (unsigned)H, (unsigned)n), a, 4.0 * W_CTX * (double)W_CTX * d * n);
         }
         if (flat) {
-            if (!launch_gemm_flat<FEPI_BF16>(c, w->attn.as<op_t>(), Wb + ly.out_w, Wf + ly.out_b, w->delta.as<op_t>(), (int)M, d, d, d, 1, 0, PCE_K_GEMM_FLAT_OUT))
-                return pce_fail(c, PCE_E_LIMIT, "attention projection does not fit the 256 x 256 kernel");
-            add_ln(ly.ln2_w, ly.ln2_b, true, false, l == 0);
-            if (!launch_gemm_flat<FEPI_GELU>(c, w->ln_out.as<op_t>(), Wb + ly.m1_w, Wf + ly.m1_b, w->hidden.as<op_t>(), (int)M, 4 * d, d, 4 * d, 1, 0, PCE_K_GEMM_FLAT_FC1) ||
-                !launch_gemm_flat<FEPI_BF16>(c, w->hidden.as<op_t>(), Wb + ly.m2_w, Wf + ly.m2_b, w->delta2.as<op_t>(), (int)M, d, 4 * d, d, 1, 0, PCE_K_GEMM_FLAT_FC2))
+            const bool ok_out = resid16 ? launch_gemm_flat<FEPI_RESID>(c, w->attn.as<op_t>(), Wb + ly.out_w, Wf + ly.out_b, w->resid16.as<op_t>(), (int)M, d, d, d, 1, 0, PCE_K_GEMM_FLAT_OUT)
+                                        : launch_gemm_flat<FEPI_BF16>(c, w->attn.as<op_t>(), Wb + ly.out_w, Wf + ly.out_b, w->delta.as<op_t>(), (int)M, d, d, d, 1, 0, PCE_K_GEMM_FLAT_OUT);
+            if (!ok_out) return pce_fail(c, PCE_E_LIMIT, "attention projection does not fit the 256 x 256 kernel");
+            add_ln(ly.ln2_w, ly.ln2_b, true, false);
+            if (!launch_gemm_flat<FEPI_GELU>(c, w->ln_out.as<op_t>(), Wb + ly.m1_w, Wf + ly.m1_b, w->hidden.as<op_t>(), (int)M, 4 * d, d, 4 * d, 1, 0, PCE_K_GEMM_FLAT_FC1))
                 return pce_fail(c, PCE_E_LIMIT, "MLP does not fit the 256 x 256 kernel");
-            if (l + 1 < L) add_ln(w->layers[(size_t)l + 1].ln1_w, w->layers[(size_t)l + 1].ln1_b, false, false, l == 0);
-            else add_ln(w->lnp_w, w->lnp_b, false, true, l == 0);
+            const bool ok_fc2 = resid16 ? launch_gemm_flat<FEPI_RESID>(c, w->hidden.as<op_t>(), Wb + ly.m2_w, Wf + ly.m2_b, w->resid16.as<op_t>(), (int)M, d, 4 * d, d, 1, 0, PCE_K_GEMM_FLAT_FC2)
+                                        : launch_gemm_flat<FEPI_BF16>(c, w->hidden.as<op_t>(), Wb + ly.m2_w, Wf + ly.m2_b, w->delta2.as<op_t>(), (int)M, d, 4 * d, d, 1, 0, PCE_K_GEMM_FLAT_FC2);
+            if (!ok_fc2) return pce_fail(c, PCE_E_LIMIT, "MLP does not fit the 256 x 256 kernel");
+            if (l + 1 < L) add_ln(w->layers[(size_t)l + 1].ln1_w, w->layers[(size_t)l + 1].ln1_b, false, false);
+            else add_ln(w->lnp_w, w->lnp_b, false, true);
             continue;
         }
         launch_gemm<EPI_RESID_F32>(c, w->attn.as<op_t>(), d, 0, Wb + ly.out_w, (int)M, d, d, Wf + ly.out_b, w->resid.as<float>(), d, 0, 1);
@@ -2387,6 +2405,32 @@
     (void)hipStreamSynchronize(c->stream);
     pce_profile_collect(c);
     return rc;
+}
+
+int pce_selftest_gemm_resid(pce_ctx *c, const uint16_t *A, const uint16_t *B, const float *bias, int32_t M, int32_t N, int32_t K, uint16_t *C)
+{
+    if (!c || !A || !B || !C || M <= 0 || N <= 0 || K <= 0) return PCE_E_INVALID;
+    PCE_HIP(c, hipSetDevice(c->device));
+    { const int rc = lds_optins(c, ws_of(c)); if (rc) return rc; }
+    const size_t rows_pad = (size_t)((M + F_T - 1) / F_T + 15) / 16 * 16 * F_T, n_c = (size_t)M * N, n_guard = (rows_pad - (size_t)M) * N;
+    DevBuf dA, dB, dC, dbias;
+    PCE_HIP(c, dA.reserve((size_t)M * K * 2)); PCE_HIP(c, dB.reserve((size_t)N * K * 2)); PCE_HIP(c, dC.reserve((n_c + n_guard) * 2)); PCE_HIP(c, dbias.reserve((size_t)N * 4));
+    PCE_HIP(c, hipMemcpyAsync(dA.p, A, (size_t)M * K * 2, hipMemcpyHostToDevice, c->stream));
+    PCE_HIP(c, hipMemcpyAsync(dB.p, B, (size_t)N * K * 2, hipMemcpyHostToDevice, c->stream));
+    if (bias) PCE_HIP(c, hipMemcpyAsync(dbias.p, bias, (size_t)N * 4, hipMemcpyHostToDevice, c->stream));
+    PCE_HIP(c, hipMemcpyAsync(dC.p, C, n_c * 2, hipMemcpyHostToDevice, c->stream));
+    PCE_HIP(c, hipMemsetAsync(dC.as<uint16_t>() + n_c, 0x5A, n_guard * 2, c->stream));
+    if (!launch_gemm_flat<FEPI_RESID>(c, dA.as<op_t>(), dB.as<op_t>(), bias ? dbias.as<float>() : nullptr, dC.as<op_t>(), M, N, K, N))
+        return pce_fail(c, PCE_E_LIMIT, "shape not handled by the 256 x 256 kernel (N %% 256, K %% 64)");
+    std::vector<uint16_t> guard(n_guard);
+    PCE_HIP(c, hipGetLastError());
+    PCE_HIP(c, hipMemcpyAsync(C, dC.p, n_c * 2, hipMemcpyDeviceToHost, c->stream));
+    PCE_HIP(c, hipMemcpyAsync(guard.data(), dC.as<uint16_t>() + n_c, n_guard * 2, hipMemcpyDeviceToHost, c->stream));
+    PCE_HIP(c, hipStreamSynchronize(c->stream));
+    pce_profile_collect(c);
+    for (size_t i = 0; i < n_guard; i++)
+        if (guard[i] != 0x5A5A) return pce_fail(c, PCE_E_DEVICE, "selftest gemm (residual epilogue): row %lld past M was written", (long long)(M + i / N));
+    return PCE_OK;
 }
 
 int pce_selftest_gemm_tiled(pce_ctx *c, int32_t kernel, int32_t epilogue, const uint16_t *A, int64_t a_len, int64_t lda, int64_t a_batch, int32_t batch,
diff --git a/prosody-control-french-tts_amd/engine.py b/prosody-control-french-tts_amd/engine.py
--- a/prosody-control-french-tts_amd/engine.py
+++ b/prosody-control-french-tts_amd/engine.py
@@ -102,7 +102,7 @@
            "pce_stft_db_run", "pce_stft_db_shape", "pce_stft_db_fetch", "pce_stft_db_device",
            "pce_resample_run", "pce_download_pcm_s16",
            "pce_dtw", "pce_dtw_series", "pce_nw_align", "pce_levenshtein", "pce_whisper_decoder_load", "pce_whisper_align_run", "pce_whisper_align_shape", "pce_whisper_align_fetch", "pce_whisper_align_paths_enqueue", "pce_whisper_align_paths_wait", "pce_whisper_sample_keys", "pce_whisper_decode_step", "pce_whisper_decode_step_ex", "pce_whisper_decode_loop", "pce_whisper_set_operands", "pce_whisper_get_operands", "pce_selftest_xattn", "pce_selftest_gemm_tiled", "pce_selftest_layernorm",
-           "pce_logmel_run", "pce_logmel_run_at", "pce_logmel_fetch", "pce_whisper_load", "pce_whisper_encode_run", "pce_selftest_gemm", "pce_selftest_attention", "pce_whisper_encode_fetch",
+           "pce_logmel_run", "pce_logmel_run_at", "pce_logmel_fetch", "pce_whisper_load", "pce_whisper_encode_run", "pce_selftest_gemm", "pce_selftest_gemm_resid", "pce_selftest_attention", "pce_whisper_encode_fetch",
            "pce_stats_enqueue", "pce_stats_wait", "pce_bert_load", "pce_bert_run", "pce_bert_fetch",
            "pce_profile_enable", "pce_profile_reset", "pce_profile_get", "pce_profile_get_work", "pce_kernel_name"]
 
@@ -172,6 +172,7 @@
     lib.pce_whisper_load.argtypes = [vp, C.POINTER(WhisperDims), vp, i64]
     lib.pce_whisper_encode_run.argtypes = [vp]
     lib.pce_selftest_gemm.argtypes = [vp, vp, vp, vp, i32, i32, i32, i32, i32, i32, vp]
+    lib.pce_selftest_gemm_resid.argtypes = [vp, vp, vp, vp, i32, i32, i32, vp]
     lib.pce_selftest_attention.argtypes = [vp, vp, vp, vp, i32, i32, i32, i32, i32, i32, vp, vp]
     lib.pce_selftest_xattn.argtypes = [vp] * 11 + [i32] * 5 + [vp]
     lib.pce_selftest_gemm_tiled.argtypes = [vp, i32, i32, vp, i64, i64, i64, i32, vp, vp, i32, i32, i32, vp, i64, i64, i64, vp, i32, i32, i32, i32, vp, i64, vp]
@@ -446,6 +447,17 @@
         if split:
             return res[:M * split].reshape(M, split), res[M * split:].reshape(M // rows_per_clip, N - split, vt_sp)
         return res.reshape(M // rows_per_clip, N, vt_sp) if epilogue == 2 else res.reshape(M, N)
+
+    def selftest_gemm_resid(self, A, B, bias, C):
+        import torch
+        a, b, cc = (torch.from_numpy(np.ascontiguousarray(x, dtype=np.float32)).to(self._op_dtype()).contiguous() for x in (A, B, C))
+        M, K = a.shape; N = b.shape[0]
+        assert cc.shape == (M, N)
+        bv = None if bias is None else np.ascontiguousarray(bias, dtype=np.float32)
+        out = cc.view(torch.int16).numpy().view(np.uint16).copy()
+        self._check(self._lib.pce_selftest_gemm_resid(self._ctx, a.view(torch.int16).numpy().ctypes.data, b.view(torch.int16).numpy().ctypes.data,
+                                                      bv.ctypes.data if bv is not None else None, M, N, K, out.ctypes.data))
+        return out
 
     def selftest_attention(self, q, k, v, causal: bool = False, mode: int = 0):
         import torch
```

Result: no change. 20650 (median of 6 runs) (+0.9%).
